# hlesmqh/WS3D

Measured on AMD Instinct MI355X. Metric: KITTI scenes/sec (16384 pts) Stage-1 RPN fwd, 1/2/4/8 GPU; FPS+group HBM GB/s, higher is better.
Workload: dtype f32

## Files before the change

### include/ws3d_ops.h

```cpp
#ifndef WS3D_OPS_H
#define WS3D_OPS_H

#include <stddef.h>
#include <stdint.h>

#ifdef __cplusplus
extern "C" {
#endif

#define WS3D_OK 0
#define WS3D_E_INVALID (-1)
#define WS3D_E_LAUNCH (-2)
#define WS3D_E_WORKSPACE (-3)
#define WS3D_E_UNSUPPORTED (-4)

#if defined(__GNUC__)
#define WS3D_API __attribute__((visibility("default")))
#else
#define WS3D_API
#endif

typedef void *ws3d_stream_t;

#define WS3D_ABI_VERSION 6
// ... 65 lines not shown
                  int32_t *idx, const void *sorted_known, ws3d_stream_t stream);

WS3D_API int ws3d_three_nn_weights(long rows, const float *dist2, float *weight, ws3d_stream_t stream);
WS3D_API int ws3d_three_nn_w(int b, int n, int m, const float *unknown, const float *known, float *dist2, int32_t *idx, float *weight,
                             const void *sorted_known, ws3d_stream_t stream);
WS3D_API int ws3d_three_nn_wq(int b, int n, int m, const float *unknown, const float *known, float *dist2, int32_t *idx, float *weight,
                              const void *sorted_known, const void *sorted_unknown, ws3d_stream_t stream);
WS3D_API int ws3d_three_nn_jobs(int b, int njobs, const int *n, const int *m, const float *const *unknown, const void *const *sorted_known,
                                float *const *dist2, int32_t *const *idx, float *const *weight, const void *const *sorted_unknown,
                                ws3d_stream_t stream);

WS3D_API int ws3d_pool_nsample(long rows, int nsample, const float *x, float *out, uint8_t *arg, ws3d_stream_t stream);
WS3D_API int ws3d_pool_nsample_grad(long rows, int nsample, const float *grad_out, const uint8_t *arg, float *grad_x,
                                    ws3d_stream_t stream);

WS3D_API int ws3d_gemm_pool(long rows, int nsample, int k_dim, int o_dim, const float *x_rows, const float *wt,
                            const float *bias, int relu, float *out, int out_stride, const int32_t *gate, long gate_limit, ws3d_stream_t stream);

WS3D_API int ws3d_gather_gemm(int b, int n, int m, int nsample, int c_feat, int o_dim, const float *feats, const float *xyz,
                     const float *new_xyz, const int32_t *nbr, const float *wt, const float *bias, int relu, float *out,
                     ws3d_stream_t stream);

WS3D_API int ws3d_gather_gemm2(int b, int n, int m, int nsample, int c_feat, int o1, int o2, const float *feats, const float *xyz,
                      const float *new_xyz, const int32_t *nbr, const float *w1t, const float *b1, int relu1, const float *w2t,
                      const float *b2, int relu2, float *out, ws3d_stream_t stream);

WS3D_API int ws3d_pgather_gemm2(int b, int n, int m, int nsample, int o1, int o2, const float *pmat, int p_stride, const float *xyz,
                       const float *new_xyz, const int32_t *nbr, const float *w1x, const float *b1, int relu1,
                       const float *w2t, const float *b2, int relu2, float *out, const int32_t *gate, long gate_limit, ws3d_stream_t stream);
WS3D_API int ws3d_pgather_rows(int b, int n, int m, int nsample, int o1, const float *pmat, int p_stride, const float *xyz, const float *new_xyz,
                      const int32_t *nbr, const float *w1x, const float *b1, int relu1, float *out, ws3d_stream_t stream);

WS3D_API int ws3d_qinterp_rows(int b, int n, int m, int o, const float *q, const int32_t *idx, const float *weight, const float *lin,
                      const float *skip, int c1, const float *wb, const float *bias, int relu, float *out, ws3d_stream_t stream);


WS3D_API int ws3d_compact_pairs(long centres, int nsample, const int32_t *nbr, int32_t *rowc, int32_t *rowsrc, int32_t *total, ws3d_stream_t stream);
WS3D_API int ws3d_compact_pairs_count(long centres, int nsample, const int32_t *nbr, int32_t *cnt, ws3d_stream_t stream);
WS3D_API int ws3d_compact_pairs_rows(long centres, int nsample, const int32_t *nbr, const int32_t *cnt, const int32_t *incl, int32_t *rowc,
                            int32_t *rowsrc, int32_t *total, ws3d_stream_t stream);
WS3D_API int ws3d_pgather_gemm2_compact(int b, int n, int m, long max_rows, int o1, int o2, const float *pmat, int p_stride, const float *xyz,
                               const float *new_xyz, const int32_t *rowc, const int32_t *rowsrc, const int32_t *total, const float *w1x,
                               const float *b1, int relu1, const float *w2t, const float *b2, int relu2, float *out, long limit, ws3d_stream_t stream);
WS3D_API int ws3d_pgather_gemm3_compact(int b, int n, int m, long max_rows, int o1, int o2, int o3, const float *pmat, int p_stride, const float *xyz,
                               const float *new_xyz, const int32_t *rowc, const int32_t *rowsrc, const int32_t *total, const float *w1x,
                               const float *b1, int relu1, const float *w2t, const float *b2, int relu2, const float *w3t, const float *b3,
                               float *out, int out_stride, long limit, ws3d_stream_t stream);
WS3D_API int ws3d_gemm_pool_compact(long max_rows, int k_dim, int o_dim, const float *x_rows, const int32_t *rowc, const int32_t *total,
                           const float *wt, const float *bias, float *out, int out_stride, long limit, ws3d_stream_t stream);
typedef struct ws3d_compact_mlp_args {
    int b, n, m;
    long max_rows;
    int o1, o2, o3;
    const float *pmat;
    int p_stride;
    const float *xyz, *new_xyz;
    const int32_t *rowc, *rowsrc, *total;
    const float *w1x, *b1;
    int relu1;
    const float *w2t, *b2;
    int relu2;
    const float *w3t, *b3;
    float *mid;
    float *out;
    int out_stride;
    long limit;
} ws3d_compact_mlp_args;
WS3D_API int ws3d_compact_mlp_pair(int kind, const ws3d_compact_mlp_args *scale0, const ws3d_compact_mlp_args *scale1, ws3d_stream_t stream);
WS3D_API int ws3d_chain_mlp3_ticket_ints(void);
WS3D_API size_t ws3d_chain_mlp3_blob_floats(int o2);
WS3D_API int ws3d_chain_mlp3_pack(const ws3d_compact_mlp_args *scale, float *blob, ws3d_stream_t stream);
WS3D_API int ws3d_chain_mlp3(const ws3d_compact_mlp_args *scale0, const ws3d_compact_mlp_args *scale1, const float *blob0, const float *blob1,
                             int32_t *ticket, int workgroups, ws3d_stream_t stream);

WS3D_API int ws3d_sa_mlp3_pool_compact(int b, int n, int m, long max_rows, int c1, int c2, int c3, const float *xyz, const float *new_xyz,
                              const float *feat, const int32_t *rowc, const int32_t *rowsrc, const int32_t *total, const float *w1t,
                              const float *b1, const float *w2t, const float *b2, const float *w3t, const float *b3, float *out,
                              int out_stride, long limit, ws3d_stream_t stream);

WS3D_API int ws3d_sa_mlp3_pool_lists(int b, int n, int m, int nsample, int c1, int c2, int c3, const float *xyz, const float *new_xyz,
                            const float *feat, const int32_t *nbr, const float *w1t, const float *b1, const float *w2t, const float *b2,
                            const float *w3t, const float *b3, int relu3, float *out, int out_stride, const int32_t *gate, long gate_limit,
                            ws3d_stream_t stream);

WS3D_API int ws3d_interp_gemm(int b, int n, int m, int c2, int c1, int o_dim, const float *known_feats, const float *unknown_feats,
                     const int32_t *idx, const float *weight, const float *wt, const float *bias, int relu, float *out,
                     ws3d_stream_t stream);

WS3D_API size_t ws3d_conv1x1_wgrad_workspace_bytes(int b, int o, int c, long l);
WS3D_API int ws3d_conv1x1_wgrad(int b, int o, int c, long l, const float *grad_out, const float *x, float *grad_w,
                                void *workspace, size_t workspace_bytes, ws3d_stream_t stream);

WS3D_API size_t ws3d_bn_workspace_bytes(int b, int c, long l);
WS3D_API int ws3d_bn_relu_train_fwd(int b, int c, long l, const float *x, const float *gamma, const float *beta, float eps,
                                    float momentum, int relu, float *running_mean, float *running_var,
                                    int64_t *num_batches_tracked, float *y, float *save_mean, float *save_invstd,
                                    void *workspace, size_t workspace_bytes, ws3d_stream_t stream);
WS3D_API int ws3d_bn_relu_train_bwd(int b, int c, long l, const float *x, const float *dy, const float *gamma,
                                    const float *beta, const float *save_mean, const float *save_invstd, int relu, float *dx,
                                    float *dgamma, float *dbeta, void *workspace, size_t workspace_bytes, ws3d_stream_t stream);

WS3D_API int ws3d_three_interpolate(int b, int c, int m, int n, const float *points, const int32_t *idx,
                           const float *weight, float *out, ws3d_stream_t stream);

WS3D_API int ws3d_three_interpolate_grad(int b, int c, int n, int m, const float *grad_out,
                                const int32_t *idx, const float *weight, float *grad_points,
                                ws3d_stream_t stream);

WS3D_API size_t ws3d_scatter_workspace_bytes(int b, int c, int n_targets, long slots_per_scene);
WS3D_API int ws3d_group_points_grad_det(int b, int c, int n, int npoints, int nsample, const float *grad_out,
                                        const int32_t *idx, float *grad_points, void *workspace,
                                        size_t workspace_bytes, ws3d_stream_t stream);
WS3D_API int ws3d_three_interpolate_grad_det(int b, int c, int n, int m, const float *grad_out, const int32_t *idx,
                                             const float *weight, float *grad_points, void *workspace,
                                             size_t workspace_bytes, ws3d_stream_t stream);

WS3D_API int ws3d_bias_act_inplace(int b, int o_ch, long l, int relu, float *y, const float *bias,
                                   ws3d_stream_t stream);

WS3D_API int ws3d_rowmax_bias_act(int b, int o_ch, long m, int s, int relu, const float *y, const float *bias,
                                  float *out, ws3d_stream_t stream);

WS3D_API int ws3d_query_and_group_nlc(int b, int n, int m, int c, float radius, int nsample, int use_xyz,
                                      const float *xyz, const float *new_xyz, const float *features_nlc,
                                      int32_t *idx_out, float *out_nlc, const void *sorted, ws3d_stream_t stream);
WS3D_API int ws3d_three_interpolate_nlc(int b, int c, int m, int n, const float *feats_nlc, const int32_t *idx,
                                        const float *weight, float *out_nlc, int out_stride, ws3d_stream_t stream);
WS3D_API int ws3d_rowmax_rows(long rows_out, int ns, int o_ch, const float *y, float *out, int out_stride,
                              ws3d_stream_t stream);

WS3D_API int ws3d_sa_mlp3_pool(long rows, int nsample, int c1, int c2, int c3, const float *x_rows4,
                               const float *w1t, const float *b1, const float *w2t, const float *b2,
                               const float *w3t, const float *b3, int relu3, float *out, int out_stride,
                               ws3d_stream_t stream);

WS3D_API int ws3d_mlp2_rows(long rows, int k_dim, int o1, int o2, const float *x_rows, const float *w1t, const float *b1, int relu1,
                   const float *w2t, const float *b2, int relu2, float *out, int *ticket, ws3d_stream_t stream);

WS3D_API size_t ws3d_rpn_heads_blob_bytes(int o2);
WS3D_API int ws3d_rpn_heads_pack(int o2, const float *w1t, const float *b1, int relu1, const float *w2t, const float *b2, int relu2, void *blob,
                        ws3d_stream_t stream);
WS3D_API int ws3d_rpn_heads(long rows, const float *x_rows, int heads, const void *blob_cls, float *out_cls, int *ticket_cls, int o2_reg,
                   const void *blob_reg, float *out_reg, int *ticket_reg, int workgroups, ws3d_stream_t stream);

WS3D_API size_t ws3d_gemm_rows_pack_bytes(int k_dim, int n_dim);
WS3D_API int ws3d_gemm_rows_pack(int k_dim, int n_dim, const float *wt, void *pack, ws3d_stream_t stream);
WS3D_API int ws3d_gemm_rows_split(long rows, int k_dim, int n_dim, const float *a, const void *pack, const float *bias, int relu, float *out,
                         ws3d_stream_t stream);

WS3D_API int ws3d_qinterp_gemm(int b, int n, int m, int c, int o_dim, const float *q, const int32_t *idx, const float *weight, const float *lin,
                      const float *skip, int c1, const float *wb, const float *b1, int relu1, const float *w2t, const float *b2, int relu2,
                      float *out, ws3d_stream_t stream);


WS3D_API int ws3d_boxes_overlap_bev(int num_a, const float *boxes_a, int num_b, const float *boxes_b,
                           float *ans, ws3d_stream_t stream);

WS3D_API int ws3d_boxes_iou_bev(int num_a, const float *boxes_a, int num_b, const float *boxes_b,
                       float *ans, ws3d_stream_t stream);

WS3D_API int ws3d_boxes_iou3d_paired(int n, const float *boxes_a, const float *boxes_b, float *overlap_bev, float *iou2d, float *iou3d,
                                     ws3d_stream_t stream);

WS3D_API int ws3d_nms_mask(int boxes_num, const float *boxes, float thresh, int normal, int full_grid,
                  uint64_t *mask, ws3d_stream_t stream);

WS3D_API size_t ws3d_nms_workspace_bytes(int boxes_num);
WS3D_API int ws3d_nms(int boxes_num, const float *boxes, float thresh, int normal, int max_keep,
                      void *workspace, size_t workspace_bytes, int64_t *keep, int32_t *num_keep,
                      ws3d_stream_t stream);

WS3D_API int ws3d_nms_batched(int batch, int boxes_num, const float *boxes, float thresh, int normal,
                              int max_keep, void *workspace, size_t workspace_bytes, int64_t *keep,
                              int32_t *num_keep, ws3d_stream_t stream);


WS3D_API int ws3d_radius_nms_batched(int batch, int n, const float *centers, float radius, int max_keep,
                                     void *workspace, size_t workspace_bytes, int64_t *keep,
                                     int32_t *num_keep, ws3d_stream_t stream);

WS3D_API int ws3d_topk_sorted(int b, int n, int k, const float *scores, float *out_scores, int64_t *out_idx,
                              ws3d_stream_t stream);
WS3D_API size_t ws3d_topk_workspace_bytes(int b, int n);
WS3D_API int ws3d_topk_sorted_ws(int b, int n, int k, const float *scores, float *out_scores, int64_t *out_idx, void *workspace,
                                 size_t workspace_bytes, ws3d_stream_t stream);
WS3D_API int ws3d_topk_sorted_sigmoid(int b, int n, int k, const float *logits, float *out_scores, int64_t *out_idx, ws3d_stream_t stream);
WS3D_API int ws3d_topk_sorted_sigmoid_ws(int b, int n, int k, const float *logits, float *out_scores, int64_t *out_idx, void *workspace,
                                         size_t workspace_bytes, ws3d_stream_t stream);

WS3D_API int ws3d_decode_center_boxes(int b, int n, int bins, float loc_scope, float loc_bin_size, float h, float w,
                                      float l, const float *xyz, const float *rpn_reg, float *boxes,
                                      ws3d_stream_t stream);

WS3D_API int ws3d_gather_boxes_bev(int b, int n, int top, const float *box, const int64_t *order, float *box_sorted, float *bev,
                          ws3d_stream_t stream);
WS3D_API int ws3d_decode_gather_boxes_bev(int b, int n, int top, int bins, float loc_scope, float loc_bin_size, float h, float w, float l,
                                          const float *xyz, const float *rpn_reg, const int64_t *order, float *box_sorted, float *bev,
                                          ws3d_stream_t stream);
WS3D_API int ws3d_select_proposals(int b, int top, int keep_stride, int k, const float *box_sorted, const float *scores_sorted,
                          const int64_t *keep, const int32_t *num, float extra_width, float *boxes_out, float *scores_out,
                          int64_t *count, float *pooled_boxes, ws3d_stream_t stream);
WS3D_API int ws3d_select_proposals_packed(int b, int top, int keep_stride, int k, const float *box_sorted, const float *scores_sorted,
                                          const int64_t *keep, const int32_t *num, float extra_width, float *boxes_out, float *scores_out,
                                          int64_t *count, float *pooled_boxes, float *packed, ws3d_stream_t stream);
WS3D_API int ws3d_select_proposals_send(int b, int top, int keep_stride, int k, const float *box_sorted, const float *scores_sorted,
                                        const int64_t *keep, const int32_t *num, float extra_width, float *boxes_out, float *scores_out,
                                        int64_t *count, float *pooled_boxes, float *send, long send_stride, ws3d_stream_t stream);
WS3D_API int ws3d_split_points_clear(long rows, int c, const float *pc, float *xyz, float *feats, void *clear, size_t clear_bytes,
                                     ws3d_stream_t stream);


WS3D_API int ws3d_roipool3d(int batch_size, int pts_num, int boxes_num, int feature_in_len,
                   int sampled_pts_num, const float *xyz, const float *boxes3d,
                   const float *pts_feature, float *pooled_features, int32_t *pooled_empty_flag,
                   int32_t *pts_idx, ws3d_stream_t stream);
WS3D_API int ws3d_roipool3d_fill(int batch_size, int pts_num, int boxes_num, int feature_in_len,
                   int sampled_pts_num, const float *xyz, const float *boxes3d,
                   const float *pts_feature, float *pooled_features, int32_t *pooled_empty_flag,
                   int32_t *pts_idx, ws3d_stream_t stream);

WS3D_API size_t ws3d_roipool3d_workspace_bytes(int batch_size, int pts_num);
WS3D_API int ws3d_roipool3d_ws(int batch_size, int pts_num, int boxes_num, int feature_in_len, int sampled_pts_num, const float *xyz,
                               const float *boxes3d, const float *pts_feature, float *pooled_features, int32_t *pooled_empty_flag,
                               int32_t *pts_idx, int fill, void *workspace, size_t workspace_bytes, ws3d_stream_t stream);


WS3D_API int ws3d_pts_in_boxes3d(int boxes_num, int pts_num, const float *pts, const float *boxes3d,
                        int64_t *flag, ws3d_stream_t stream);


WS3D_API int ws3d_instance_clouds(int batch, int pts_num, int centres_num, int feat_len, int sampled_pts_num, float radius, int mask_mode,
                                  float mask_thresh, const float *pts, const float *score, const float *feats, const float *centres,
                                  const int32_t *num, float *cloud, float *cloud_feats, int32_t *count, int32_t *pts_idx,
                                  ws3d_stream_t stream);
WS3D_API int ws3d_instance_clouds_count(int batch, int pts_num, int centres_num, float radius, const float *pts, const float *centres,
                                        const int32_t *num, int32_t *count, ws3d_stream_t stream);
WS3D_API int ws3d_instance_clouds_emit(int batch, int pts_num, int centres_num, int feat_len, float radius, int mask_mode, float mask_thresh,
                                       const float *pts, const float *score, const float *feats, const float *centres, const int32_t *num,
                                       const int64_t *offsets, float *rows, float *row_feats, int32_t *row_idx, ws3d_stream_t stream);


WS3D_API int ws3d_click_prepare(int batch, int pts_num, int clicks_num, int side, const float *offsets, float gauss_height, float gauss_status,
                                float gauss_cov, float centre_y, const float *pts, const float *clicks, const int32_t *num, float *score,
                                float *cand, int32_t *cand_num, ws3d_stream_t stream);



WS3D_API int ws3d_kitti_overlaps(int metric, int criterion, int frames, long max_pairs, const int32_t *gt_off, const int32_t *dt_off,
                                 const int64_t *out_off, const double *dt_boxes, const double *gt_boxes, double *out,
                                 ws3d_stream_t stream);

WS3D_API int ws3d_kitti_collect_scores(int frames, int max_dt, const int32_t *gt_off, const int32_t *dt_off, const int64_t *out_off,
                                       const double *overlaps, const int32_t *ignored_gt, const int32_t *ignored_dt,
                                       const double *dt_score, double min_overlap, double *tp_score, int32_t *tp_flag,
                                       ws3d_stream_t stream);

WS3D_API size_t ws3d_kitti_count_workspace_bytes(int frames, int num_thresh);
WS3D_API int ws3d_kitti_count(int metric, int frames, int max_dt, int num_thresh, const double *thresholds, const int32_t *gt_off,
                              const int32_t *dt_off, const int32_t *dc_off, const int64_t *out_off, const double *overlaps,
                              const int32_t *ignored_gt, const int32_t *ignored_dt, const double *dt_score, const double *dt_alpha,
                              const double *gt_alpha, const double *dt_bbox, const double *dc_bbox, double min_overlap, int compute_aos,
                              void *workspace, size_t workspace_bytes, double *pr, ws3d_stream_t stream);


WS3D_API int ws3d_stage2_embed(long rows, int pts_per_cloud, const float *pts, const float *box_ce, float extend, const float *wx0,
                               const float *bx0, const float *wx1, const float *bx1, const float *wf0, const float *bf0, const float *wf1,
                               const float *bf1, const float *wm, const float *bm, float *xyz_out, float *feat, ws3d_stream_t stream);
WS3D_API int ws3d_stage2_boxes(int rows, int loc_bins, int head_bins, float loc_scope, float h, float w, float l, const float *rcnn_reg,
                               float *pred_boxes3d, float *box_ce, ws3d_stream_t stream);
WS3D_API int ws3d_stage2_select(int batch, int slots, float cls_thresh, float iou_thresh, const float *size_window, float ground_y,
                                const float *box_ce, const float *rcnn_ref, const float *rcnn_cls, const float *rcnn_iou, const float *center,
                                const int32_t *num, float *boxes, int32_t *keep, float *key, ws3d_stream_t stream);

WS3D_API int ws3d_stage2_canonical_ragged(int rows, int clouds, const int32_t *offsets, const float *pts, const float *box_ce, float extend,
                                          float *pts_out, ws3d_stream_t stream);
WS3D_API int ws3d_furthest_point_sampling_ragged_gather(int clouds, const int32_t *offsets, const int32_t *sizes_host, int m, const float *xyz,
                                                        int32_t *idx, float *new_xyz, ws3d_stream_t stream);
WS3D_API int ws3d_ball_query_ragged(int clouds, const int32_t *offsets, int m, float radius, int nsample, const float *xyz, const float *new_xyz,
                                    int global_rows, int32_t *idx, ws3d_stream_t stream);

WS3D_API int ws3d_stage2_rcnn_loss(int rows, int loc_bins, int head_bins, float loc_scope, float h, float w, float l, const float *rcnn_cls,
                                   const float *rcnn_reg, const float *pred_boxes3d, const float *gt_boxes, const float *cls, float *vals,
                                   int32_t *counts, float *grad_cls, float *grad_reg, ws3d_stream_t stream);
WS3D_API int ws3d_stage2_ioun_loss(int rows, const float *rcnn_iou, const float *rcnn_ref, const float *pred_boxes3d, const float *refined_box,
                                   const float *gt_boxes, const float *cls, float *vals, int32_t *counts, float *grad_iou, float *grad_ref,
                                   ws3d_stream_t stream);

WS3D_API int ws3d_rpn_center_labels(int batch, int n, int kmax, int pts_stride, float gauss_height, float gauss_status, double gauss_cov,
                                    const float *pts, const float *centres, const int32_t *count, float *cls_label, float *reg_label,
                                    ws3d_stream_t stream);
WS3D_API size_t ws3d_rpn_loss_workspace_bytes(int rows);
WS3D_API int ws3d_rpn_loss(int rows, int bins, double loc_scope, double loc_bin_size, double alpha, double gamma, double weight_cls,
                           double weight_reg, const float *rpn_cls, const float *rpn_reg, const float *cls_label, const float *reg_label,
                           float *vals, int32_t *counts, float *grad_cls, float *grad_reg, void *workspace, size_t workspace_bytes,
                           ws3d_stream_t stream);

WS3D_API int ws3d_scan_prepare_limit(void);
WS3D_API size_t ws3d_scan_prepare_workspace_bytes(int scenes, long total_points);
WS3D_API int ws3d_scan_prepare(int scenes, const int32_t *offsets, long total_points, int max_scan_points, const float *raw, const float *calib,
                               const int32_t *img_hw, const float *scope, int npoints, uint64_t seed, const int64_t *scene_key, int key_bits,
                               float *pts_input, int32_t *src_index, int32_t *valid_count, int32_t *status, void *workspace,
                               size_t workspace_bytes, ws3d_stream_t stream);

WS3D_API int ws3d_stage2_batch_param_bytes(void);
WS3D_API int ws3d_stage2_batch(int samples, const void *params, const float *rows, const int32_t *offsets, int records, long total_rows,
                               int key_bits, float *cur_box_point, float *cur_box_reflect, float *train_mask, int32_t *status,
// ... 14 lines not shown
```

### ws3d_amd/_lib.py

```python
from __future__ import annotations

import ctypes as C
import os

_HERE = os.path.dirname(os.path.abspath(__file__))
DIST_MODE = int(os.environ.get("WS3D_DIST_MODE", "0") or 0)
LIB_PATH = os.environ.get("WS3D_HIP_LIB") or os.path.join(
    _HERE, "libws3d_hip.so" if DIST_MODE == 0 else "libws3d_hip_dm%d.so" % DIST_MODE)

E_INVALID, E_LAUNCH, E_WORKSPACE, E_UNSUPPORTED = -1, -2, -3, -4
ABI_VERSION = 6

_vp = C.c_void_p
_i = C.c_int
_f = C.c_float
_sz = C.c_size_t

class CompactMlpArgs(C.Structure):
    _fields_ = [("b", _i), ("n", _i), ("m", _i), ("max_rows", C.c_long), ("o1", _i), ("o2", _i), ("o3", _i), ("pmat", _vp), ("p_stride", _i),
                ("xyz", _vp), ("new_xyz", _vp), ("rowc", _vp), ("rowsrc", _vp), ("total", _vp), ("w1x", _vp), ("b1", _vp), ("relu1", _i),
                ("w2t", _vp), ("b2", _vp), ("relu2", _i), ("w3t", _vp), ("b3", _vp), ("mid", _vp), ("out", _vp), ("out_stride", _i), ("limit", C.c_long)]


SIGNATURES = {
    "ws3d_abi_version": (_i, []),
    "ws3d_tune": (_i, [_i, _i]),
    "ws3d_dist_mode": (_i, []),
    "ws3d_last_error": (C.c_char_p, []),
    "ws3d_device_info": (_i, [C.c_char_p, _i, C.POINTER(_i), C.POINTER(_i)]),
    "ws3d_furthest_point_sampling": (_i, [_i, _i, _i, _vp, _vp, _vp, _vp]),
    "ws3d_furthest_point_sampling_gather": (_i, [_i, _i, _i, _vp, _vp, _vp, _vp, _vp]),
    "ws3d_furthest_point_sampling_nested": (_i, [_i, _i, _i, _vp, _vp, _vp, _vp]),
    "ws3d_furthest_point_sampling_nested_chain": (_i, [_i, _i, _i, _vp, _vp, _vp, _vp, _vp]),
    "ws3d_fps_ragged_limit": (_i, []),
    "ws3d_furthest_point_sampling_ragged": (_i, [_i, _vp, _vp, _i, _vp, _vp, _vp]),
    "ws3d_fps_workspace_bytes": (_sz, [_i, _i]),
    "ws3d_furthest_point_sampling_ws": (_i, [_i, _i, _i, _vp, _vp, _vp, _vp, _vp, _sz, _vp]),
    "ws3d_gather_points": (_i, [_i, _i, _i, _i, _vp, _vp, _vp, _vp]),
    "ws3d_gather_points_grad": (_i, [_i, _i, _i, _i, _vp, _vp, _vp, _vp]),
    "ws3d_ball_query": (_i, [_i, _i, _i, _f, _i, _vp, _vp, _vp, _vp, _vp]),
    "ws3d_ball_query_fill": (_i, [_i, _i, _i, _f, _i, _vp, _vp, _vp, _vp, _vp]),
    "ws3d_ball_query_pairs": (_i, [_i, _i, _i, _f, _i, _vp, _vp, _vp, _vp, _vp, _vp, _vp, _vp]),
    "ws3d_ball_query_pairs2": (_i, [_i, _i, _i, _vp, _vp, _vp, C.c_float, _i, _vp, _vp, _vp, _vp, C.c_float, _i, _vp, _vp, _vp, _vp, _vp]),
    "ws3d_sorted_points_bytes": (_sz, [_i, _i]),
    "ws3d_sort_points_x": (_i, [_i, _i, _vp, _vp, _vp]),
    "ws3d_sort_points_xz": (_i, [_i, _i, _vp, _vp, _vp]),
    "ws3d_sort_points_grid": (_i, [_i, _i, _vp, _vp, _vp]),
    "ws3d_sort_points_jobs": (_i, [_i, _i, _vp, _vp, _vp, _vp, _vp]),
    "ws3d_group_points": (_i, [_i, _i, _i, _i, _i, _vp, _vp, _vp, _vp]),
    "ws3d_group_points_grad": (_i, [_i, _i, _i, _i, _i, _vp, _vp, _vp, _vp]),
    "ws3d_query_and_group": (_i, [_i, _i, _i, _i, _f, _i, _i, _vp, _vp, _vp, _vp, _vp, _vp, _vp]),
    "ws3d_three_nn": (_i, [_i, _i, _i, _vp, _vp, _vp, _vp, _vp, _vp]),
    "ws3d_three_interpolate": (_i, [_i, _i, _i, _i, _vp, _vp, _vp, _vp, _vp]),
    "ws3d_three_interpolate_grad": (_i, [_i, _i, _i, _i, _vp, _vp, _vp, _vp, _vp]),
    "ws3d_bn_workspace_bytes": (C.c_size_t, [_i, _i, C.c_long]),
    "ws3d_bn_relu_train_fwd": (_i, [_i, _i, C.c_long, _vp, _vp, _vp, C.c_float, C.c_float, _i, _vp, _vp, _vp, _vp, _vp, _vp,
                                    _vp, C.c_size_t, _vp]),
    "ws3d_bn_relu_train_bwd": (_i, [_i, _i, C.c_long, _vp, _vp, _vp, _vp, _vp, _vp, _i, _vp, _vp, _vp, _vp, C.c_size_t, _vp]),
    "ws3d_conv1x1_wgrad_workspace_bytes": (C.c_size_t, [_i, _i, _i, C.c_long]),
    "ws3d_conv1x1_wgrad": (_i, [_i, _i, _i, C.c_long, _vp, _vp, _vp, _vp, C.c_size_t, _vp]),
    "ws3d_gemm_pool": (_i, [C.c_long, _i, _i, _i, _vp, _vp, _vp, _i, _vp, _i, _vp, C.c_long, _vp]),
    "ws3d_pool_nsample": (_i, [C.c_long, _i, _vp, _vp, _vp, _vp]),
    "ws3d_pool_nsample_grad": (_i, [C.c_long, _i, _vp, _vp, _vp, _vp]),
    "ws3d_scatter_workspace_bytes": (C.c_size_t, [_i, _i, _i, C.c_long]),
    "ws3d_group_points_grad_det": (_i, [_i, _i, _i, _i, _i, _vp, _vp, _vp, _vp, C.c_size_t, _vp]),
    "ws3d_three_interpolate_grad_det": (_i, [_i, _i, _i, _i, _vp, _vp, _vp, _vp, _vp, C.c_size_t, _vp]),
    "ws3d_query_and_group_nlc": (_i, [_i, _i, _i, _i, _f, _i, _i, _vp, _vp, _vp, _vp, _vp, _vp, _vp]),
    "ws3d_three_interpolate_nlc": (_i, [_i, _i, _i, _i, _vp, _vp, _vp, _vp, _i, _vp]),
    "ws3d_rowmax_rows": (_i, [C.c_long, _i, _i, _vp, _vp, _i, _vp]),
    "ws3d_sa_mlp3_pool": (_i, [C.c_long, _i, _i, _i, _i, _vp, _vp, _vp, _vp, _vp, _vp, _vp, _i, _vp, _i, _vp]),
    "ws3d_qinterp_gemm": (_i, [_i, _i, _i, _i, _i, _vp, _vp, _vp, _vp, _vp, _i, _vp, _vp, _i, _vp, _vp, _i, _vp, _vp]),
    "ws3d_mlp2_rows": (_i, [C.c_long, _i, _i, _i, _vp, _vp, _vp, _i, _vp, _vp, _i, _vp, _vp, _vp]),
    "ws3d_rpn_heads_blob_bytes": (_sz, [_i]),
    "ws3d_rpn_heads_pack": (_i, [_i, _vp, _vp, _i, _vp, _vp, _i, _vp, _vp]),
    "ws3d_rpn_heads": (_i, [C.c_long, _vp, _i, _vp, _vp, _vp, _i, _vp, _vp, _vp, _i, _vp]),
    "ws3d_gemm_rows_pack_bytes": (_sz, [_i, _i]),
    "ws3d_gemm_rows_pack": (_i, [_i, _i, _vp, _vp, _vp]),
    "ws3d_gemm_rows_split": (_i, [C.c_long, _i, _i, _vp, _vp, _vp, _i, _vp, _vp]),
    "ws3d_decode_center_boxes": (_i, [_i, _i, _i, _f, _f, _f, _f, _f, _vp, _vp, _vp, _vp]),
    "ws3d_topk_sorted": (_i, [_i, _i, _i, _vp, _vp, _vp, _vp]),
    "ws3d_topk_workspace_bytes": (C.c_size_t, [_i, _i]),
    "ws3d_topk_sorted_ws": (_i, [_i, _i, _i, _vp, _vp, _vp, _vp, C.c_size_t, _vp]),
    "ws3d_topk_sorted_sigmoid": (_i, [_i, _i, _i, _vp, _vp, _vp, _vp]),
    "ws3d_topk_sorted_sigmoid_ws": (_i, [_i, _i, _i, _vp, _vp, _vp, _vp, C.c_size_t, _vp]),
    "ws3d_three_nn_weights": (_i, [C.c_long, _vp, _vp, _vp]),
    "ws3d_three_nn_w": (_i, [_i, _i, _i, _vp, _vp, _vp, _vp, _vp, _vp, _vp]),
    "ws3d_three_nn_wq": (_i, [_i, _i, _i, _vp, _vp, _vp, _vp, _vp, _vp, _vp, _vp]),
    "ws3d_three_nn_jobs": (_i, [_i, _i, _vp, _vp, _vp, _vp, _vp, _vp, _vp, _vp, _vp]),
    "ws3d_bias_act_inplace": (_i, [_i, _i, C.c_long, _i, _vp, _vp, _vp]),
    "ws3d_rowmax_bias_act": (_i, [_i, _i, C.c_long, _i, _i, _vp, _vp, _vp, _vp]),
    "ws3d_boxes_overlap_bev": (_i, [_i, _vp, _i, _vp, _vp, _vp]),
    "ws3d_boxes_iou_bev": (_i, [_i, _vp, _i, _vp, _vp, _vp]),
    "ws3d_boxes_iou3d_paired": (_i, [_i, _vp, _vp, _vp, _vp, _vp, _vp]),
    "ws3d_nms_mask": (_i, [_i, _vp, _f, _i, _i, _vp, _vp]),
    "ws3d_nms_workspace_bytes": (_sz, [_i]),
    "ws3d_nms": (_i, [_i, _vp, _f, _i, _i, _vp, _sz, _vp, _vp, _vp]),
    "ws3d_nms_batched": (_i, [_i, _i, _vp, _f, _i, _i, _vp, _sz, _vp, _vp, _vp]),
    "ws3d_radius_nms_batched": (_i, [_i, _i, _vp, _f, _i, _vp, _sz, _vp, _vp, _vp]),
    "ws3d_gather_gemm": (_i, [_i, _i, _i, _i, _i, _i, _vp, _vp, _vp, _vp, _vp, _vp, _i, _vp, _vp]),
    "ws3d_gather_gemm2": (_i, [_i, _i, _i, _i, _i, _i, _i, _vp, _vp, _vp, _vp, _vp, _vp, _i, _vp, _vp, _i, _vp, _vp]),
    "ws3d_pgather_gemm2": (_i, [_i, _i, _i, _i, _i, _i, _vp, _i, _vp, _vp, _vp, _vp, _vp, _i, _vp, _vp, _i, _vp, _vp, C.c_long, _vp]),
    "ws3d_pgather_rows": (_i, [_i, _i, _i, _i, _i, _vp, _i, _vp, _vp, _vp, _vp, _vp, _i, _vp, _vp]),
    "ws3d_qinterp_rows": (_i, [_i, _i, _i, _i, _vp, _vp, _vp, _vp, _vp, _i, _vp, _vp, _i, _vp, _vp]),
    "ws3d_compact_pairs": (_i, [C.c_long, _i, _vp, _vp, _vp, _vp, _vp]),
    "ws3d_compact_pairs_count": (_i, [C.c_long, _i, _vp, _vp, _vp]),
    "ws3d_compact_pairs_rows": (_i, [C.c_long, _i, _vp, _vp, _vp, _vp, _vp, _vp, _vp]),
    "ws3d_pgather_gemm2_compact": (_i, [_i, _i, _i, C.c_long, _i, _i, _vp, _i, _vp, _vp, _vp, _vp, _vp, _vp, _vp, _i, _vp, _vp, _i, _vp, C.c_long, _vp]),
    "ws3d_pgather_gemm3_compact": (_i, [_i, _i, _i, C.c_long, _i, _i, _i, _vp, _i, _vp, _vp, _vp, _vp, _vp, _vp, _vp, _i, _vp, _vp, _i, _vp, _vp, _vp, _i, C.c_long, _vp]),
    "ws3d_gemm_pool_compact": (_i, [C.c_long, _i, _i, _vp, _vp, _vp, _vp, _vp, _vp, _i, C.c_long, _vp]),
    "ws3d_compact_mlp_pair": (_i, [_i, C.POINTER(CompactMlpArgs), C.POINTER(CompactMlpArgs), _vp]),
    "ws3d_chain_mlp3_ticket_ints": (_i, []),
    "ws3d_chain_mlp3_blob_floats": (_sz, [_i]),
    "ws3d_chain_mlp3_pack": (_i, [C.POINTER(CompactMlpArgs), _vp, _vp]),
    "ws3d_chain_mlp3": (_i, [C.POINTER(CompactMlpArgs), C.POINTER(CompactMlpArgs), _vp, _vp, _vp, _i, _vp]),
    "ws3d_sa_mlp3_pool_compact": (_i, [_i, _i, _i, C.c_long, _i, _i, _i, _vp, _vp, _vp, _vp, _vp, _vp, _vp, _vp, _vp, _vp, _vp, _vp, _vp, _i, C.c_long, _vp]),
    "ws3d_sa_mlp3_pool_lists": (_i, [_i, _i, _i, _i, _i, _i, _i, _vp, _vp, _vp, _vp, _vp, _vp, _vp, _vp, _vp, _vp, _i, _vp, _i, _vp, C.c_long, _vp]),
    "ws3d_interp_gemm": (_i, [_i, _i, _i, _i, _i, _i, _vp, _vp, _vp, _vp, _vp, _vp, _i, _vp, _vp]),
    "ws3d_gather_boxes_bev": (_i, [_i, _i, _i, _vp, _vp, _vp, _vp, _vp]),
    "ws3d_select_proposals": (_i, [_i, _i, _i, _i, _vp, _vp, _vp, _vp, _f, _vp, _vp, _vp, _vp, _vp]),
    "ws3d_decode_gather_boxes_bev": (_i, [_i, _i, _i, _i, _f, _f, _f, _f, _f, _vp, _vp, _vp, _vp, _vp, _vp]),
    "ws3d_select_proposals_packed": (_i, [_i, _i, _i, _i, _vp, _vp, _vp, _vp, _f, _vp, _vp, _vp, _vp, _vp, _vp]),
    "ws3d_select_proposals_send": (_i, [_i, _i, _i, _i, _vp, _vp, _vp, _vp, _f, _vp, _vp, _vp, _vp, _vp, C.c_long, _vp]),
    "ws3d_split_points_clear": (_i, [C.c_long, _i, _vp, _vp, _vp, _vp, C.c_size_t, _vp]),
    "ws3d_roipool3d": (_i, [_i, _i, _i, _i, _i, _vp, _vp, _vp, _vp, _vp, _vp, _vp]),
    "ws3d_roipool3d_fill": (_i, [_i, _i, _i, _i, _i, _vp, _vp, _vp, _vp, _vp, _vp, _vp]),
    "ws3d_roipool3d_workspace_bytes": (C.c_size_t, [_i, _i]),
    "ws3d_roipool3d_ws": (_i, [_i, _i, _i, _i, _i, _vp, _vp, _vp, _vp, _vp, _vp, _i, _vp, C.c_size_t, _vp]),
    "ws3d_pts_in_boxes3d": (_i, [_i, _i, _vp, _vp, _vp, _vp]),
    "ws3d_instance_clouds": (_i, [_i, _i, _i, _i, _i, _f, _i, _f, _vp, _vp, _vp, _vp, _vp, _vp, _vp, _vp, _vp, _vp]),
    "ws3d_instance_clouds_count": (_i, [_i, _i, _i, _f, _vp, _vp, _vp, _vp, _vp]),
    "ws3d_instance_clouds_emit": (_i, [_i, _i, _i, _i, _f, _i, _f, _vp, _vp, _vp, _vp, _vp, _vp, _vp, _vp, _vp, _vp]),
    "ws3d_click_prepare": (_i, [_i, _i, _i, _i, _vp, _f, _f, _f, _f, _vp, _vp, _vp, _vp, _vp, _vp, _vp]),
    "ws3d_kitti_overlaps": (_i, [_i, _i, _i, C.c_long, _vp, _vp, _vp, _vp, _vp, _vp, _vp]),
    "ws3d_kitti_collect_scores": (_i, [_i, _i, _vp, _vp, _vp, _vp, _vp, _vp, _vp, C.c_double, _vp, _vp, _vp]),
    "ws3d_kitti_count_workspace_bytes": (_sz, [_i, _i]),
    "ws3d_kitti_count": (_i, [_i, _i, _i, _i, _vp, _vp, _vp, _vp, _vp, _vp, _vp, _vp, _vp, _vp, _vp, _vp, _vp, C.c_double, _i, _vp,
                              _sz, _vp, _vp]),
    "ws3d_stage2_embed": (_i, [C.c_long, _i, _vp, _vp, _f] + [_vp] * 10 + [_vp, _vp, _vp]),
    "ws3d_stage2_boxes": (_i, [_i, _i, _i, _f, _f, _f, _f, _vp, _vp, _vp, _vp]),
    "ws3d_stage2_select": (_i, [_i, _i, _f, _f, C.POINTER(_f), _f, _vp, _vp, _vp, _vp, _vp, _vp, _vp, _vp, _vp, _vp]),
    "ws3d_stage2_canonical_ragged": (_i, [_i, _i, _vp, _vp, _vp, _f, _vp, _vp]),
    "ws3d_furthest_point_sampling_ragged_gather": (_i, [_i, _vp, _vp, _i, _vp, _vp, _vp, _vp]),
    "ws3d_ball_query_ragged": (_i, [_i, _vp, _i, _f, _i, _vp, _vp, _i, _vp, _vp]),
    "ws3d_stage2_rcnn_loss": (_i, [_i, _i, _i, _f, _f, _f, _f] + [_vp] * 9 + [_vp]),
    "ws3d_stage2_ioun_loss": (_i, [_i] + [_vp] * 10 + [_vp]),
    "ws3d_rpn_center_labels": (_i, [_i, _i, _i, _i, _f, _f, C.c_double] + [_vp] * 5 + [_vp]),
    "ws3d_rpn_loss_workspace_bytes": (_sz, [_i]),
    "ws3d_rpn_loss": (_i, [_i, _i] + [C.c_double] * 6 + [_vp] * 8 + [_vp, _sz, _vp]),
    "ws3d_scan_prepare_limit": (_i, []),
    "ws3d_scan_prepare_workspace_bytes": (_sz, [_i, C.c_long]),
    "ws3d_scan_prepare": (_i, [_i, _vp, C.c_long, _i, _vp, _vp, _vp, _vp, _i, C.c_uint64, _vp, _i, _vp, _vp, _vp, _vp, _vp, _sz, _vp]),
    "ws3d_stage2_batch_param_bytes": (_i, []),
    "ws3d_stage2_batch": (_i, [_i, _vp, _vp, _vp, _i, C.c_long, _i, _vp, _vp, _vp, _vp, _vp]),
    "ws3d_roipool3d_plan": (_i, [_i, _i, _i, _i, _i, _i, _sz]),
    "ws3d_ball_query_plan": (_i, [_i, _i, _i, _i, _i, _i, _i, _i, _i, _i, _i, _vp]),
}


class Ws3dError(RuntimeError):
    pass


_lib = None


def load() -> C.CDLL:
    global _lib
    if _lib is not None:
        return _lib
    if not os.path.exists(LIB_PATH):
        raise Ws3dError(
            f"{LIB_PATH} is missing: the MI355X HIP library has not been built "
            "(run `python -m ws3d_amd.build`).  ws3d_amd has no CPU fallback.")
    import torch
    try:
        lib = C.CDLL(LIB_PATH)
    except OSError as e:
        raise Ws3dError(f"cannot load {LIB_PATH}: {e}") from e
    for name, (res, args) in SIGNATURES.items():
        fn = getattr(lib, name)
        fn.restype = res
        fn.argtypes = args
    if lib.ws3d_abi_version() != ABI_VERSION:
        raise Ws3dError(f"{LIB_PATH} exports ABI version {lib.ws3d_abi_version()}, this package binds version {ABI_VERSION}: "
                        "rebuild it (`python -m ws3d_amd.build`)")
    if not os.environ.get("WS3D_HIP_LIB") and lib.ws3d_dist_mode() != DIST_MODE:
        raise Ws3dError(f"{LIB_PATH} was built with WS3D_DIST_MODE={lib.ws3d_dist_mode()}, expected {DIST_MODE}: rebuild it")
    _lib = lib
    return lib


def check(rc: int, what: str = "") -> None:
    if rc != 0:
        msg = load().ws3d_last_error()
        raise Ws3dError(f"{what or 'ws3d'} failed (rc={rc}): {msg.decode() if msg else ''}")
```

### ws3d_amd/build.py

```python
from __future__ import annotations

import argparse
import concurrent.futures as cf
import glob
import os
import shutil
import subprocess
import sys

HERE = os.path.dirname(os.path.abspath(__file__))
CSRC = os.path.join(HERE, "csrc")
OBJ = os.path.join(CSRC, "build")
LIB = os.path.join(HERE, "libws3d_hip.so")
DIST_MODES = (0, 1, 2)


def lib_path(dist_mode: int = 0) -> str:
    return LIB if dist_mode == 0 else os.path.join(HERE, "libws3d_hip_dm%d.so" % dist_mode)
ARCH = "gfx950"
SOURCES = ["core.hip", "fps.hip", "fps_v3.hip", "fps_bucket.hip", "fps_nested.hip", "fps_ragged.hip", "fps_pruned.hip", "ballquery_group.hip", "interpolate.hip", "roipool3d.hip", "iou3d.hip", "proposals.hip", "scatter_det.hip", "sa_mlp.hip", "bn_relu.hip", "gemm_pool.hip", "conv_wgrad.hip", "chain_mlp.hip", "rpn_heads.hip", "gemm_rows.hip", "kitti_eval.hip", "instance_clouds.hip", "click.hip", "stage2.hip", "stage2_ragged.hip", "stage2_loss.hip", "rpn_targets.hip", "scan_prepare.hip", "stage2_batch.hip"]
CXXFLAGS = ["-O3", "-std=c++17", "-fPIC", "-ffp-contract=off", "-fno-fast-math",
            "-fvisibility=hidden", "-Wall", "-Wno-unused-function"]


def hipcc() -> str:
    for cand in (os.environ.get("HIPCC"), shutil.which("hipcc"), "/opt/rocm/bin/hipcc"):
        if cand and os.path.exists(cand):
            return cand
    raise RuntimeError("hipcc not found (looked at $HIPCC, PATH, /opt/rocm/bin)")


def _deps(src: str):
    return [src, *glob.glob(os.path.join(CSRC, "*.h")), os.path.join(HERE, "..", "include", "ws3d_ops.h"),
            os.path.join(CSRC, "exports.map"), os.path.abspath(__file__)]


def _compile(src: str, force: bool, verbose: bool, dist_mode: int = 0) -> str:
    path = os.path.join(CSRC, src)
    obj = os.path.join(OBJ if dist_mode == 0 else OBJ + "_dm%d" % dist_mode, os.path.splitext(src)[0] + ".o")
    if not force and os.path.exists(obj) and all(
            os.path.getmtime(obj) >= os.path.getmtime(d) for d in _deps(path)):
        return obj
    cmd = [hipcc(), f"--offload-arch={ARCH}", *CXXFLAGS, f"-DWS3D_DIST_MODE={dist_mode}", *os.environ.get("WS3D_EXTRA_DEFS", "").split(), "-c", path, "-o", obj]
    if verbose:
        print(" ".join(cmd), flush=True)
    r = subprocess.run(cmd, capture_output=True, text=True)
    if r.returncode != 0:
        raise RuntimeError(f"hipcc failed for {src}:\n{r.stdout}\n{r.stderr}")
    if verbose and r.stderr.strip():
        print(r.stderr)
    return obj


def build(force: bool = False, verbose: bool = False, dist_mode: int = 0) -> str:
    LIB = lib_path(dist_mode)
    os.makedirs(OBJ if dist_mode == 0 else OBJ + "_dm%d" % dist_mode, exist_ok=True)
    with cf.ThreadPoolExecutor(max_workers=min(len(SOURCES), os.cpu_count() or 4, 16)) as ex:
        objs = list(ex.map(lambda s: _compile(s, force, verbose, dist_mode), SOURCES))
    if force or not os.path.exists(LIB) or any(os.path.getmtime(o) > os.path.getmtime(LIB) for o in objs):
        cmd = [hipcc(), f"--offload-arch={ARCH}", "-shared", "-fPIC", "-Wl,--version-script=" + os.path.join(CSRC, "exports.map"), "-o", LIB, *objs]
        if verbose:
            print(" ".join(cmd), flush=True)
        r = subprocess.run(cmd, capture_output=True, text=True)
        if r.returncode != 0:
            raise RuntimeError(f"link failed:\n{r.stdout}\n{r.stderr}")
    return LIB


def rebuild_one(src: str, verbose: bool = False) -> str:
    _compile(src, True, verbose)
    objs = [os.path.join(OBJ, os.path.splitext(s_)[0] + ".o") for s_ in SOURCES]
    missing = [o for o in objs if not os.path.exists(o)]
    if missing:
        return build(False, verbose)
    cmd = [hipcc(), f"--offload-arch={ARCH}", "-shared", "-fPIC", "-Wl,--version-script=" + os.path.join(CSRC, "exports.map"), "-o", LIB, *objs]
    r = subprocess.run(cmd, capture_output=True, text=True)
    if r.returncode != 0:
        raise RuntimeError(f"link failed:\n{r.stdout}\n{r.stderr}")
    return LIB


if __name__ == "__main__":
    ap = argparse.ArgumentParser()
    ap.add_argument("--force", action="store_true")
    ap.add_argument("--verbose", action="store_true")
    ap.add_argument("--dist-mode", type=int, default=0, choices=DIST_MODES)
    ap.add_argument("--all-dist-modes", action="store_true")
    ap.add_argument("--only", default=None, help="recompile this one source (forced) and relink")
    a = ap.parse_args()
    if a.only:
        print(rebuild_one(a.only, a.verbose))
        sys.exit(0)
    for dm in (DIST_MODES if a.all_dist_modes else (a.dist_mode,)):
        print(build(a.force, a.verbose, dm))
    sys.exit(0)
```

### ws3d_amd/compat.py

```python
from __future__ import annotations

import sys
import types

import os

import torch

from . import _lib
from ._lib import Ws3dError, check


def _dev(*tensors):
    dev = None
    for t in tensors:
        if t is None:
            continue
        if not t.is_cuda:
            raise Ws3dError("ws3d_amd ops need HIP ('cuda') tensors; there is no CPU fallback")
        if not t.is_contiguous():
            raise Ws3dError("ws3d_amd ops need contiguous tensors (the reference asserts the same)")
        if dev is None:
            dev = t.device
        elif t.device != dev:
# ... 388 lines not shown
    b, c = x.size(0), x.size(1)
    l = x.numel() // max(b * c, 1)
    y = torch.empty_like(x)
    mean = torch.empty((c,), dtype=torch.float32, device=dev)
    invstd = torch.empty((c,), dtype=torch.float32, device=dev)
    lib = _lib.load()
    nbytes = lib.ws3d_bn_workspace_bytes(b, c, l)
    ws = torch.empty((nbytes + 7) // 8, dtype=torch.float64, device=dev)
    with _on(dev):
        check(lib.ws3d_bn_relu_train_fwd(b, c, l, _p(x), _p(gamma), _p(beta), float(eps), float(momentum), int(bool(relu)),
                                         _p(running_mean), _p(running_var), _p(num_batches_tracked), _p(y), _p(mean), _p(invstd), _p(ws), nbytes,
                                         _stream()), "bn_relu_train_fwd")
    return y, mean, invstd


def bn_relu_train_bwd(x, dy, gamma, beta, save_mean, save_invstd, relu=True):
    dev = _dev(x, dy, gamma, beta, save_mean, save_invstd)
    _f32(x, "x"); _f32(dy, "dy")
    b, c = x.size(0), x.size(1)
    l = x.numel() // max(b * c, 1)
    dx = torch.empty_like(x)
    dgamma = torch.empty((c,), dtype=torch.float32, device=dev)
    dbeta = torch.empty((c,), dtype=torch.float32, device=dev)
    lib = _lib.load()
    nbytes = lib.ws3d_bn_workspace_bytes(b, c, l)
    ws = torch.empty((nbytes + 7) // 8, dtype=torch.float64, device=dev)
    with _on(dev):
        check(lib.ws3d_bn_relu_train_bwd(b, c, l, _p(x), _p(dy), _p(gamma), _p(beta), _p(save_mean), _p(save_invstd),
                                         int(bool(relu)), _p(dx), _p(dgamma), _p(dbeta), _p(ws), nbytes, _stream()),
              "bn_relu_train_bwd")
    return dx, dgamma, dbeta


def conv1x1_wgrad(grad_out, x, shape=None):
    dev = _dev(grad_out, x)
    _f32(grad_out, "grad_out"); _f32(x, "x")
    b, o, c = x.size(0), grad_out.size(1), x.size(1)
    l = x.numel() // max(b * c, 1)
    if grad_out.numel() != b * o * l:
        raise Ws3dError("conv1x1_wgrad: grad_out and x disagree in shape")
    gw = torch.empty((o, c) if shape is None else tuple(shape), dtype=torch.float32, device=dev)
    lib = _lib.load()
    nbytes = lib.ws3d_conv1x1_wgrad_workspace_bytes(b, o, c, l)
    ws = torch.empty((nbytes + 3) // 4, dtype=torch.float32, device=dev)
    with _on(dev):
        check(lib.ws3d_conv1x1_wgrad(b, o, c, l, _p(grad_out), _p(x), _p(gw), _p(ws), nbytes, _stream()), "conv1x1_wgrad")
    return gw


def _gate(gate):
    if gate is None:
        return None, 0
    total, limit = gate
    return total.data_ptr(), int(limit)


def gemm_pool(x_rows, wt, bias, relu, nsample, out, col0=0, gate=None):
    dev = _dev(x_rows, wt, bias)
    _f32(x_rows, "x_rows"); _f32(wt, "wt")
    rows, k = x_rows.shape
    o = wt.size(1)
    if rows % 64 or rows // 64 > 65535 or o % 64 or k % 4 or nsample not in (16, 32) or wt.size(0) != k:
        return False
    view = out[:, col0:col0 + o]
    with _on(dev):
        check(_lib.load().ws3d_gemm_pool(rows, nsample, k, o, _p(x_rows), _p(wt), _p(bias), int(bool(relu)), view.data_ptr(),
                                         out.size(1), *_gate(gate), _stream()), "gemm_pool")
    return True


def gather_gemm(feats, xyz, new_xyz, nbr, wt_feat_then_xyz, bias, relu):
    dev = _dev(feats, xyz, new_xyz, nbr, wt_feat_then_xyz)
    _f32(feats, "feats"); _f32(xyz, "xyz"); _f32(new_xyz, "new_xyz"); _i32(nbr, "nbr"); _f32(wt_feat_then_xyz, "wt")
    B, N, C = feats.shape
    M, ns = nbr.size(1), nbr.size(2)
    O = wt_feat_then_xyz.size(1)
    rows = B * M * ns
    if C % 4 or O % 64 or rows % 64 or rows // 64 > 65535 or wt_feat_then_xyz.size(0) != C + 3 or not feats.is_contiguous():
        return None
    out = torch.empty((rows, O), dtype=torch.float32, device=dev)
    with _on(dev):
        check(_lib.load().ws3d_gather_gemm(B, N, M, ns, C, O, _p(feats), _p(xyz), _p(new_xyz), _p(nbr), _p(wt_feat_then_xyz), _p(bias),
                                           int(bool(relu)), _p(out), _stream()), "gather_gemm")
    return out


def gather_gemm2(feats, xyz, new_xyz, nbr, w1t_feat_then_xyz, b1, relu1, w2t, b2, relu2):
    dev = _dev(feats, xyz, new_xyz, nbr, w1t_feat_then_xyz, w2t)
    _f32(feats, "feats"); _f32(xyz, "xyz"); _f32(new_xyz, "new_xyz"); _i32(nbr, "nbr"); _f32(w1t_feat_then_xyz, "w1t"); _f32(w2t, "w2t")
    B, N, C = feats.shape
    M, ns = nbr.size(1), nbr.size(2)
    O1, O2 = w1t_feat_then_xyz.size(1), w2t.size(1)
    rows = B * M * ns
    if (C % 4 or O1 not in (64, 128, 256) or O2 % 4 or rows % 64 or w1t_feat_then_xyz.size(0) != C + 3 or w2t.size(0) != O1 or
            not feats.is_contiguous() or not w2t.is_contiguous() or not w1t_feat_then_xyz.is_contiguous()):
        return None
    out = torch.empty((rows, O2), dtype=torch.float32, device=dev)
    with _on(dev):
        check(_lib.load().ws3d_gather_gemm2(B, N, M, ns, C, O1, O2, _p(feats), _p(xyz), _p(new_xyz), _p(nbr), _p(w1t_feat_then_xyz), _p(b1),
                                            int(bool(relu1)), _p(w2t), _p(b2), int(bool(relu2)), _p(out), _stream()), "gather_gemm2")
    return out


def pgather_gemm2(pmat, col0, o1, xyz, new_xyz, nbr, w1x, b1, relu1, w2t, b2, relu2, out=None, gate=None):
    dev = _dev(pmat, xyz, new_xyz, nbr, w1x, w2t)
    _f32(pmat, "pmat"); _f32(xyz, "xyz"); _f32(new_xyz, "new_xyz"); _i32(nbr, "nbr"); _f32(w1x, "w1x"); _f32(w2t, "w2t")
    B, N = xyz.size(0), xyz.size(1)
    M, ns = nbr.size(1), nbr.size(2)
    O2 = w2t.size(1)
    if (o1 not in (64, 128) or O2 % 4 or (M * ns) % 64 or pmat.dim() != 2 or pmat.size(0) != B * N or pmat.stride(1) != 1 or
            col0 < 0 or col0 + o1 > pmat.size(1) or tuple(w1x.shape) != (3, o1) or w2t.size(0) != o1 or not w1x.is_contiguous() or not w2t.is_contiguous()):
        return None
    if out is None:
        out = torch.empty((B * M * ns, O2), dtype=torch.float32, device=dev)
    elif tuple(out.shape) != (B * M * ns, O2) or not out.is_contiguous():
        raise ValueError("pgather_gemm2: out must be a contiguous (B*M*ns, O2) tensor")
    with _on(dev):
        check(_lib.load().ws3d_pgather_gemm2(B, N, M, ns, o1, O2, pmat.data_ptr() + 4 * col0, pmat.stride(0), _p(xyz), _p(new_xyz), _p(nbr), _p(w1x), _p(b1),
                                             int(bool(relu1)), _p(w2t), _p(b2), int(bool(relu2)), _p(out), *_gate(gate), _stream()), "pgather_gemm2")
    return out


def pgather_rows(pmat, col0, o1, xyz, new_xyz, nbr, w1x, b1, relu1):
    dev = _dev(pmat, xyz, new_xyz, nbr, w1x)
    _f32(pmat, "pmat"); _f32(xyz, "xyz"); _f32(new_xyz, "new_xyz"); _i32(nbr, "nbr"); _f32(w1x, "w1x")
    B, N = xyz.size(0), xyz.size(1)
    M, ns = nbr.size(1), nbr.size(2)
    if (o1 % 4 or col0 % 4 or pmat.dim() != 2 or pmat.size(0) != B * N or pmat.stride(1) != 1 or pmat.stride(0) % 4 or col0 < 0 or
            col0 + o1 > pmat.size(1) or tuple(w1x.shape) != (3, o1) or not w1x.is_contiguous() or pmat.data_ptr() % 16):
        return None
    out = torch.empty((B * M * ns, o1), dtype=torch.float32, device=dev)
    with _on(dev):
        check(_lib.load().ws3d_pgather_rows(B, N, M, ns, o1, pmat.data_ptr() + 4 * col0, pmat.stride(0), _p(xyz), _p(new_xyz), _p(nbr), _p(w1x), _p(b1),
                                            int(bool(relu1)), _p(out), _stream()), "pgather_rows")
    return out


def qinterp_rows(q, idx, weight, lin=None, skip=None, wb=None, bias=None, relu=True):
    dev = _dev(q, idx, weight)
    _f32(q, "q"); _i32(idx, "idx"); _f32(weight, "weight")
    B, M, O = q.shape
    N = idx.size(1)
    c1 = 0 if skip is None else skip.size(2)
    if (O % 4 or not q.is_contiguous() or (lin is None and c1 > 4) or (lin is not None and (tuple(lin.shape) != (B * N, O) or not lin.is_contiguous())) or
            (lin is None and c1 > 0 and (wb is None or tuple(wb.shape) != (c1, O) or not wb.is_contiguous() or not skip.is_contiguous()))):
        return None
    out = torch.empty((B * N, O), dtype=torch.float32, device=dev)
    with _on(dev):
        check(_lib.load().ws3d_qinterp_rows(B, N, M, O, _p(q), _p(idx), _p(weight), _p(lin), _p(skip), c1, _p(wb), _p(bias), int(bool(relu)), _p(out),
                                            _stream()), "qinterp_rows")
    return out


def qinterp_gemm(q, idx, weight, w2t, b2, relu2, lin=None, skip=None, wb=None, bias=None, relu=True):
    dev = _dev(q, idx, weight, w2t)
    _f32(q, "q"); _i32(idx, "idx"); _f32(weight, "weight"); _f32(w2t, "w2t")
    B, M, C = q.shape
    N = idx.size(1)
    O = w2t.size(1)
    c1 = 0 if skip is None else skip.size(2)
    if ((B * N) % 64 or C % 16 or O % 128 or w2t.size(0) != C or not q.is_contiguous() or not w2t.is_contiguous() or not idx.is_contiguous() or
            not weight.is_contiguous() or (lin is None and c1 > 4) or (lin is not None and (tuple(lin.shape) != (B * N, C) or not lin.is_contiguous())) or
            (lin is None and c1 > 0 and (wb is None or tuple(wb.shape) != (c1, C) or not wb.is_contiguous() or not skip.is_contiguous()))):
        return None
    out = torch.empty((B * N, O), dtype=torch.float32, device=dev)
    with _on(dev):
        check(_lib.load().ws3d_qinterp_gemm(B, N, M, C, O, _p(q), _p(idx), _p(weight), _p(lin), _p(skip), c1, _p(wb), _p(bias), int(bool(relu)), _p(w2t),
                                            _p(b2), int(bool(relu2)), _p(out), _stream()), "qinterp_gemm")
    return out


def compact_pairs(nbr, ordered=False):
    if not ordered:
        dev = _dev(nbr)
        _i32(nbr, "nbr")
        B, M, ns = nbr.shape
        rowc = torch.empty(B * M * ns, dtype=torch.int32, device=dev)
        rowsrc = torch.empty(B * M * ns, dtype=torch.int32, device=dev)
        total = torch.zeros(1, dtype=torch.int32, device=dev)
        with _on(dev):
            check(_lib.load().ws3d_compact_pairs(B * M, ns, _p(nbr), _p(rowc), _p(rowsrc), _p(total), _stream()), "compact_pairs")
        return rowc, rowsrc, total
    dev = _dev(nbr)
    _i32(nbr, "nbr")
    B, M, ns = nbr.shape
    centres = B * M
    cnt = torch.empty(centres, dtype=torch.int32, device=dev)
    rowc = torch.empty(centres * ns, dtype=torch.int32, device=dev)
    rowsrc = torch.empty(centres * ns, dtype=torch.int32, device=dev)
    total = torch.empty(1, dtype=torch.int32, device=dev)
    with _on(dev):
        lib = _lib.load()
        check(lib.ws3d_compact_pairs_count(centres, ns, _p(nbr), _p(cnt), _stream()), "compact_pairs_count")
        incl = torch.cumsum(cnt, dim=0, dtype=torch.int32)
        check(lib.ws3d_compact_pairs_rows(centres, ns, _p(nbr), _p(cnt), _p(incl), _p(rowc), _p(rowsrc), _p(total), _stream()), "compact_pairs_rows")
    return rowc, rowsrc, total


def pgather_gemm2_compact(pmat, col0, o1, xyz, new_xyz, pairs, w1x, b1, relu1, w2t, b2, relu2, limit=-1):
    rowc, rowsrc, total = pairs
    dev = _dev(pmat, xyz, new_xyz, rowc, w1x, w2t)
    _f32(pmat, "pmat"); _f32(xyz, "xyz"); _f32(new_xyz, "new_xyz"); _f32(w1x, "w1x"); _f32(w2t, "w2t")
    B, N = xyz.size(0), xyz.size(1)
    M = new_xyz.size(1)
    O2 = w2t.size(1)
    rows = rowc.numel()
    if (o1 not in (64, 128, 256) or O2 % 4 or pmat.dim() != 2 or pmat.size(0) != B * N or pmat.stride(1) != 1 or col0 < 0 or col0 + o1 > pmat.size(1) or
            tuple(w1x.shape) != (3, o1) or w2t.size(0) != o1 or not w1x.is_contiguous() or not w2t.is_contiguous()):
        return None
    out = torch.empty((rows, O2), dtype=torch.float32, device=dev)
    with _on(dev):
        check(_lib.load().ws3d_pgather_gemm2_compact(B, N, M, rows, o1, O2, pmat.data_ptr() + 4 * col0, pmat.stride(0), _p(xyz), _p(new_xyz), _p(rowc),
                                                     _p(rowsrc), _p(total), _p(w1x), _p(b1), int(bool(relu1)), _p(w2t), _p(b2), int(bool(relu2)), _p(out),
                                                     int(limit), _stream()), "pgather_gemm2_compact")
    return out


def pgather_gemm3_compact(pmat, col0, o1, xyz, new_xyz, pairs, w1x, b1, relu1, w2t, b2, relu2, w3t, b3, out2d, col_offset, limit=-1, max_lds=160 * 1024):
    rowc, rowsrc, total = pairs
    dev = _dev(pmat, xyz, new_xyz, rowc, w1x, w2t, w3t, out2d)
    _f32(pmat, "pmat"); _f32(xyz, "xyz"); _f32(new_xyz, "new_xyz"); _f32(w1x, "w1x"); _f32(w2t, "w2t"); _f32(w3t, "w3t"); _f32(out2d, "out2d")
    B, N = xyz.size(0), xyz.size(1)
    M = new_xyz.size(1)
    O2, O3 = w2t.size(1), w3t.size(1)
    rows = rowc.numel()
    lds = 4 * ((o1 + (O2 + 15) // 16 * 16) * 65 + 2 * 16 * 64)
    if (o1 not in (64, 128) or O2 % 4 or O3 % 128 or lds > min(max_lds, 160 * 1024 - 1024) or pmat.dim() != 2 or pmat.size(0) != B * N or pmat.stride(1) != 1 or
            col0 < 0 or col0 + o1 > pmat.size(1) or tuple(w1x.shape) != (3, o1) or w2t.size(0) != o1 or w3t.size(0) != O2 or not w1x.is_contiguous() or
            not w2t.is_contiguous() or not w3t.is_contiguous() or out2d.dim() != 2 or out2d.stride(1) != 1 or col_offset < 0 or col_offset + O3 > out2d.size(1)):
        return False
    with _on(dev):
        check(_lib.load().ws3d_pgather_gemm3_compact(B, N, M, rows, o1, O2, O3, pmat.data_ptr() + 4 * col0, pmat.stride(0), _p(xyz), _p(new_xyz), _p(rowc),
                                                     _p(rowsrc), _p(total), _p(w1x), _p(b1), int(bool(relu1)), _p(w2t), _p(b2), int(bool(relu2)), _p(w3t), _p(b3),
                                                     out2d.data_ptr() + 4 * col_offset, out2d.stride(0), int(limit), _stream()), "pgather_gemm3_compact")
    return True


def gemm_pool_compact(x_rows, pairs, wt, bias, out2d, col_offset, limit=-1):
    rowc, rowsrc, total = pairs
    dev = _dev(x_rows, rowc, wt, out2d)
    _f32(x_rows, "x_rows"); _f32(wt, "wt"); _f32(out2d, "out2d")
    rows, k = x_rows.shape
    o = wt.size(1)
    if (k % 4 or o % 64 or wt.size(0) != k or rows != rowc.numel() or not x_rows.is_contiguous() or not wt.is_contiguous() or out2d.dim() != 2 or
            out2d.stride(1) != 1 or col_offset < 0 or col_offset + o > out2d.size(1)):
        return False
    with _on(dev):
        check(_lib.load().ws3d_gemm_pool_compact(rows, k, o, _p(x_rows), _p(rowc), _p(total), _p(wt), _p(bias), out2d.data_ptr() + 4 * col_offset,
                                                 out2d.stride(0), int(limit), _stream()), "gemm_pool_compact")
    return True


def compact_mlp_pair(kind, scales, max_lds=160 * 1024, mids=None):
    import ctypes as C
    if len(scales) != 2 or scales[0]["o1"] != scales[1]["o1"]:
        return None if kind == 2 else False
    blocks, keep, outs = [], [], []
    for si, a in enumerate(scales):
        rowc, rowsrc, total = a["pairs"]
        pmat, xyz, new_xyz, w1x, w2t, w3t, out2d, o1, col0, col = a["pmat"], a["xyz"], a["new_xyz"], a["w1x"], a["w2t"], a["w3t"], a["out2d"], a["o1"], a["col0"], a["col_offset"]
        dev = _dev(pmat, xyz, new_xyz, rowc, w1x, w2t, w3t, out2d)
        for t_, nm in ((pmat, "pmat"), (xyz, "xyz"), (new_xyz, "new_xyz"), (w1x, "w1x"), (w2t, "w2t"), (w3t, "w3t"), (out2d, "out2d")):
            _f32(t_, nm)
        B, N, M = xyz.size(0), xyz.size(1), new_xyz.size(1)
        O2, O3 = w2t.size(1), w3t.size(1)
        rows = rowc.numel()
        lds3 = 4 * ((o1 + (O2 + 15) // 16 * 16) * 65 + 2 * 16 * 64)
        ok = (O2 % 4 == 0 and pmat.dim() == 2 and pmat.size(0) == B * N and pmat.stride(1) == 1 and col0 >= 0 and col0 + o1 <= pmat.size(1) and
              tuple(w1x.shape) == (3, o1) and w2t.size(0) == o1 and w3t.size(0) == O2 and w1x.is_contiguous() and w2t.is_contiguous() and w3t.is_contiguous() and
              out2d.dim() == 2 and out2d.stride(1) == 1 and col >= 0 and col + O3 <= out2d.size(1))
        if kind == 3:
            ok = ok and o1 in (64, 128) and O3 % 128 == 0 and lds3 <= min(max_lds, 160 * 1024 - 1024)
        elif kind == 2:
            ok = ok and o1 in (64, 128, 256)
        else:
            ok = ok and O3 % 64 == 0 and mids is not None and tuple(mids[si].shape) == (rows, O2) and mids[si].is_contiguous()
        if not ok:
            return None if kind == 2 else False
        mid = mids[si] if kind == 1 else (torch.empty((rows, O2), dtype=torch.float32, device=dev) if kind == 2 else None)
        outs.append(mid)
        keep.append((pmat, xyz, new_xyz, rowc, rowsrc, total, w1x, w2t, w3t, out2d, mid, a["b1"], a["b2"], a["b3"]))
        blocks.append(_lib.CompactMlpArgs(B, N, M, rows, o1, O2, O3, pmat.data_ptr() + 4 * col0, pmat.stride(0), _p(xyz), _p(new_xyz), _p(rowc), _p(rowsrc),
                                          _p(total), _p(w1x), _p(a["b1"]), int(bool(a["relu1"])), _p(w2t), _p(a["b2"]), int(bool(a["relu2"])), _p(w3t), _p(a["b3"]),
                                          _p(mid), out2d.data_ptr() + 4 * col, out2d.stride(0), -1))
    with _on(dev):
        rc = _lib.load().ws3d_compact_mlp_pair(int(kind), C.byref(blocks[0]), C.byref(blocks[1]), _stream())
    if rc == _lib.E_UNSUPPORTED:
        return None if kind == 2 else False
    check(rc, "compact_mlp_pair")
    return outs if kind == 2 else True


CHAIN_WORKGROUPS = 0
TUNE_KEYS = {"chain_wgs": 0, "mlp2_wgs": 1, "sa1_wgs": 2, "fp_wgs": 3, "pair_wgs": 4, "bq_wide_nw": 5}


def tune(name: str, value: int = -1) -> int:
    rc = _lib.load().ws3d_tune(TUNE_KEYS[name], int(value))
    if rc < 0:
        check(rc, "tune")
    return rc


_CHAIN_BLOBS = {}


def chain_ticket_ints() -> int:
    return int(_lib.load().ws3d_chain_mlp3_ticket_ints())


def _chain_blob(block, tensors, dev):
    import ctypes as C
    key = tuple((t.data_ptr(), t._version) if t is not None else None for t in tensors)
    hit = _CHAIN_BLOBS.get(key)
    if hit is None:
        n = int(_lib.load().ws3d_chain_mlp3_blob_floats(block.o2))
        blob = torch.empty(n, dtype=torch.float32, device=dev)
        with _on(dev):
            check(_lib.load().ws3d_chain_mlp3_pack(C.byref(block), _p(blob), _stream()), "chain_mlp3_pack")
        if torch.cuda.is_current_stream_capturing():
            return blob
# ... 955 lines not shown
```

### ws3d_amd/csrc/gemm_pool.hip

```cpp
#include <cstdlib>

#include "common.h"
#include "compact_pool.h"
#include "mfma_tile.h"

namespace ws3d {

template <int NS, int MB, int NB>
__global__ __launch_bounds__(256) void gemm_pool_big_kernel(int k_dim, int o_dim, const float *__restrict__ x,
                                                            const float *__restrict__ wt, const float *__restrict__ bias,
                                                            int relu, float *__restrict__ out, int out_stride, int xcd,
                                                            const int32_t *__restrict__ gate, long gate_limit) {
    if (gate && (long)*gate <= gate_limit) return;
    constexpr int TM = 64 * MB, TN = 64 * NB;
    __shared__ float xs[2][GP_KT][TM + 1];
    __shared__ __attribute__((aligned(16))) float ws[2][GP_KT][TN];
    const Wave w;
    long row_tile;
    int col_tile;
    gg_tile<false>(o_dim / TN, xcd, blockIdx.x, row_tile, col_tile);
    const long row0 = row_tile * TM;
    const int col0 = col_tile * TN;
    RowsA<MB> load_a;
    load_a.k_dim = k_dim;
#pragma unroll
    for (int i = 0; i < MB; ++i) load_a.p[i] = x + (row0 + (w.tid >> 2) + 64 * i) * (long)k_dim;
    floatx16 acc[MB][NB];
    mfma_k_loop<MB, NB, false>(w, acc, xs, ws, k_dim, load_a, wt, o_dim, col0);
#pragma unroll
    for (int i = 0; i < MB; ++i)
#pragma unroll
        for (int j = 0; j < NB; ++j)
            pool_rows<NS>(w, acc[i][j], bias, relu, out, out_stride, row0 + sub_row<MB>(w, i), col0 + sub_col<NB, false>(w, j) + w.l32);
}

struct GatherA {
    const float *frow, *prow, *crow;
    int c_feat;
    __device__ __forceinline__ GatherA(long r, int c_feat_, int n, int m, int ns, const float *__restrict__ feats, const float *__restrict__ xyz,
                                       const float *__restrict__ new_xyz, const int32_t *__restrict__ nbr) {
        const long cm = r / ns;
        const long b = cm / m;
        const int src = nbr[r];
        frow = feats + ((size_t)b * n + (size_t)src) * c_feat_;
        prow = xyz + ((size_t)b * n + (size_t)src) * 3;
        crow = new_xyz + (size_t)cm * 3;
        c_feat = c_feat_;
    }
    __device__ __forceinline__ float4 operator()(int, int k) const {
        if (k < c_feat) return *reinterpret_cast<const float4 *>(frow + k);
        if (k == c_feat) return make_float4(prow[0] - crow[0], prow[1] - crow[1], prow[2] - crow[2], 0.f);
        return f4_zero();
    }
};

__global__ __launch_bounds__(256) void gather_gemm_kernel(int c_feat, int o_dim, int n, int m, int ns, const float *__restrict__ feats,
                                                          const float *__restrict__ xyz, const float *__restrict__ new_xyz,
                                                          const int32_t *__restrict__ nbr, const float *__restrict__ wt,
                                                          const float *__restrict__ bias, int relu, float *__restrict__ out, int tps) {
    __shared__ float xs[2][GP_KT][GP_XS];
    __shared__ __attribute__((aligned(16))) float ws[2][GP_KT][64];
    const Wave w;
    long row_tile;
    int col_tile;
    gg_tile<true>(o_dim / 64, tps, blockIdx.x, row_tile, col_tile);
    const long row0 = row_tile * 64;
    const int col0 = col_tile * 64;
    const GatherA load_a(row0 + (w.tid >> 2), c_feat, n, m, ns, feats, xyz, new_xyz, nbr);
    floatx16 acc[1][1];
    mfma_k_loop<1, 1, false>(w, acc, xs, ws, c_feat + 3, load_a, wt, o_dim, col0);
    store_rows(w, acc[0][0], bias, relu, out, o_dim, row0 + w.wm * 32, col0 + w.bc);
}

template <int NB1>
__global__ __launch_bounds__(256) void gather_gemm2_kernel(int c_feat, int o2, int n, int m, int ns, const float *__restrict__ feats,
                                                           const float *__restrict__ xyz, const float *__restrict__ new_xyz,
                                                           const int32_t *__restrict__ nbr, const float *__restrict__ w1t,
                                                           const float *__restrict__ b1, int relu1, const float *__restrict__ w2t,
                                                           const float *__restrict__ b2, int relu2, float *__restrict__ out) {
    constexpr int O1 = NB1 * 64;
    extern __shared__ __attribute__((aligned(16))) float smem2[];
    auto &xs = *reinterpret_cast<float (*)[2][GP_KT][GP_XS]>(smem2);
    auto &w1s = *reinterpret_cast<float (*)[2][GP_KT][O1]>(smem2 + 2 * GP_KT * GP_XS);
    float *act = smem2, *w2s = smem2 + O1 * GP_XS;
    const Wave w;
    const long row0 = (long)blockIdx.x * 64;
    const GatherA load_a(row0 + (w.tid >> 2), c_feat, n, m, ns, feats, xyz, new_xyz, nbr);
    floatx16 acc1[1][NB1];
    mfma_k_loop<1, NB1, true>(w, acc1, xs, w1s, c_feat + 3, load_a, w1t, O1, 0);
#pragma unroll
    for (int j = 0; j < NB1; ++j) store_act(w, acc1[0][j], b1, relu1, act, j * 64 + w.bc);
    lds_layer<1>(w, act, O1 / GP_KT, w2t, O1, o2, w2s, 0, 1, [&](const floatx16 &acc, int col) __attribute__((always_inline)) {
        if (col < o2) store_rows(w, acc, b2, relu2, out, o2, row0 + w.wm * 32, col);
    });
}

template <int NB1>
__global__ __launch_bounds__(256) void pgather_gemm2_kernel(int o2, int n, int m, int ns, const float *__restrict__ pmat, int p_stride,
                                                            const float *__restrict__ xyz, const float *__restrict__ new_xyz,
                                                            const int32_t *__restrict__ nbr, const float *__restrict__ w1x,
                                                            const float *__restrict__ b1, int relu1, const float *__restrict__ w2t,
                                                            const float *__restrict__ b2, int relu2, float *__restrict__ out,
                                                            const int32_t *__restrict__ gate, long gate_limit) {
    if (gate && (long)*gate <= gate_limit) return;
    constexpr int O1 = NB1 * 64;
    extern __shared__ __attribute__((aligned(16))) float smem2[];
    float *act = smem2, *w2s = smem2 + O1 * GP_XS;
    const Wave w;
    const long row0 = (long)blockIdx.x * 64;
    const long scene = row0 / ((long)m * ns);
    ppoint_layer1<NB1>(w, [&](int tr) __attribute__((always_inline)) { return PairRow{scene, (row0 + tr) / ns, nbr[row0 + tr]}; }, n, pmat, p_stride, xyz, new_xyz, w1x, b1, relu1, act);
    lds_layer<1>(w, act, O1 / GP_KT, w2t, O1, o2, w2s, 0, 1, [&](const floatx16 &acc, int col) __attribute__((always_inline)) {
        if (col < o2) store_rows(w, acc, b2, relu2, out, o2, row0 + w.wm * 32, col);
    });
}

__global__ __launch_bounds__(256) void pgather_rows_kernel(long rows, int o1, int n, int m, int ns, const float *__restrict__ pmat, int p_stride,
                                                           const float *__restrict__ xyz, const float *__restrict__ new_xyz,
                                                           const int32_t *__restrict__ nbr, const float *__restrict__ w1x,
                                                           const float *__restrict__ b1, int relu1, float *__restrict__ out) {
    const int q4 = o1 >> 2;
    const long total = rows * q4;
    for (long e = (long)blockIdx.x * 256 + threadIdx.x; e < total; e += (long)gridDim.x * 256) {
        const long r = e / q4;
        const int c4 = (int)(e - r * q4) * 4;
        const long cm = r / ns, scene = cm / m;
        const int src = nbr[r];
        const float *pr = xyz + ((size_t)scene * n + (size_t)src) * 3, *cr = new_xyz + (size_t)cm * 3;
        const float dx = pr[0] - cr[0], dy = pr[1] - cr[1], dz = pr[2] - cr[2];
        const float4 pv = *reinterpret_cast<const float4 *>(pmat + ((size_t)scene * n + (size_t)src) * p_stride + c4);
        const float4 wx = *reinterpret_cast<const float4 *>(w1x + c4), wy = *reinterpret_cast<const float4 *>(w1x + o1 + c4),
                     wz = *reinterpret_cast<const float4 *>(w1x + 2 * o1 + c4);
        const float4 bv = b1 ? *reinterpret_cast<const float4 *>(b1 + c4) : make_float4(0.f, 0.f, 0.f, 0.f);
        float4 y;
        y.x = __builtin_fmaf(dz, wz.x, __builtin_fmaf(dy, wy.x, __builtin_fmaf(dx, wx.x, pv.x))) + bv.x;
        y.y = __builtin_fmaf(dz, wz.y, __builtin_fmaf(dy, wy.y, __builtin_fmaf(dx, wx.y, pv.y))) + bv.y;
        y.z = __builtin_fmaf(dz, wz.z, __builtin_fmaf(dy, wy.z, __builtin_fmaf(dx, wx.z, pv.z))) + bv.z;
        y.w = __builtin_fmaf(dz, wz.w, __builtin_fmaf(dy, wy.w, __builtin_fmaf(dx, wx.w, pv.w))) + bv.w;
        if (relu1) { y.x = y.x < 0.f ? 0.f : y.x; y.y = y.y < 0.f ? 0.f : y.y; y.z = y.z < 0.f ? 0.f : y.z; y.w = y.w < 0.f ? 0.f : y.w; }
        *reinterpret_cast<float4 *>(out + r * (long)o1 + c4) = y;
    }
}

__global__ __launch_bounds__(256) void pair_count_kernel(long centres, int ns, const int32_t *__restrict__ nbr, int32_t *__restrict__ cnt) {
    const long c = (long)blockIdx.x * 256 + threadIdx.x;
    if (c >= centres) return;
    const int32_t *row = nbr + c * ns;
    int k = 1, prev = row[0];
    for (int s2 = 1; s2 < ns; ++s2) { const int v = row[s2]; k += v > prev; prev = v; }
    cnt[c] = k;
}

__global__ __launch_bounds__(256) void pair_rows_kernel(long centres, int ns, const int32_t *__restrict__ nbr, const int32_t *__restrict__ cnt,
                                                        const int32_t *__restrict__ incl, int32_t *__restrict__ rowc, int32_t *__restrict__ rowsrc,
                                                        int32_t *__restrict__ total) {
    const long e = (long)blockIdx.x * 256 + threadIdx.x;
    if (e >= centres * ns) return;
// ... 30 lines not shown
        for (int s2 = 0; s2 < k; ++s2) { rowc[first + s2] = (int32_t)c; rowsrc[first + s2] = row[s2]; }
    }
}

struct CompactSrc {
    const int32_t *__restrict__ rowc, *__restrict__ rowsrc;
    long row0, T;
    int m;
    __device__ __forceinline__ PairRow operator()(int tr) const {
        const long t = min(row0 + tr, T - 1);
        const int cm = rowc[t];
        return PairRow{cm / m, cm, rowsrc[t]};
    }
};

template <int NB1>
__device__ __forceinline__ void pgather_gemm2_compact_body(const unsigned bx, const unsigned by, const unsigned gy, int o2, int n, int m,
                                                           const float *__restrict__ pmat, int p_stride,
                                                           const float *__restrict__ xyz, const float *__restrict__ new_xyz,
                                                           const int32_t *__restrict__ rowc, const int32_t *__restrict__ rowsrc,
                                                           const int32_t *__restrict__ total, const float *__restrict__ w1x,
                                                           const float *__restrict__ b1, int relu1, const float *__restrict__ w2t,
                                                           const float *__restrict__ b2, int relu2, float *__restrict__ out, long limit) {
    constexpr int O1 = NB1 * 64;
    const long T = *total;
    const long row0 = (long)bx * 64;
    if (row0 >= T || (limit >= 0 && T > limit)) return;
    extern __shared__ __attribute__((aligned(16))) float smem2[];
    float *act = smem2, *w2s = smem2 + O1 * GP_XS;
    const Wave w;
    ppoint_layer1<NB1>(w, CompactSrc{rowc, rowsrc, row0, T, m}, n, pmat, p_stride, xyz, new_xyz, w1x, b1, relu1, act);
    lds_layer<1>(w, act, O1 / GP_KT, w2t, O1, o2, w2s, (int)by, (int)gy, [&](const floatx16 &acc, int col) __attribute__((always_inline)) {
        if (col < o2) store_rows(w, acc, b2, relu2, out, o2, row0 + w.wm * 32, col, T);
    });
}

template <int NB1>
__global__ __launch_bounds__(256) void pgather_gemm2_compact_kernel(int o2, int n, int m, const float *__restrict__ pmat, int p_stride,
                                                                    const float *__restrict__ xyz, const float *__restrict__ new_xyz,
                                                                    const int32_t *__restrict__ rowc, const int32_t *__restrict__ rowsrc,
                                                                    const int32_t *__restrict__ total, const float *__restrict__ w1x,
                                                                    const float *__restrict__ b1, int relu1, const float *__restrict__ w2t,
                                                                    const float *__restrict__ b2, int relu2, float *__restrict__ out, long limit) {
    pgather_gemm2_compact_body<NB1>(blockIdx.x, blockIdx.y, gridDim.y, o2, n, m, pmat, p_stride, xyz, new_xyz, rowc, rowsrc, total, w1x, b1, relu1, w2t, b2,
                                    relu2, out, limit);
}

struct CompactMlpArgs {
    const float *pmat, *xyz, *new_xyz;
    const int32_t *rowc, *rowsrc, *total;
    const float *w1x, *b1, *w2t, *b2, *w3t, *b3;
    float *mid, *out;
    long limit;
    int o2, o3, n, m, p_stride, relu1, relu2, out_stride, gy, pad;
};

template <int NB1>
__global__ __launch_bounds__(256) void pgather_gemm2_compact_pair_kernel(const CompactMlpArgs a0, const CompactMlpArgs a1, const unsigned split,
                                                                         const unsigned total_x) {
    for (unsigned bx = blockIdx.x; bx < total_x; bx += gridDim.x) {
        const bool second = bx >= split;
        const CompactMlpArgs &a = second ? a1 : a0;
        if (blockIdx.y < (unsigned)a.gy)
            pgather_gemm2_compact_body<NB1>(second ? bx - split : bx, blockIdx.y, (unsigned)a.gy, a.o2, a.n, a.m, a.pmat, a.p_stride, a.xyz, a.new_xyz,
                                            a.rowc, a.rowsrc, a.total, a.w1x, a.b1, a.relu1, a.w2t, a.b2, a.relu2, a.mid, a.limit);
        __syncthreads();
    }
}

__device__ __forceinline__ void gemm_pool_compact_body(const unsigned bx, int k_dim, int o_dim, const float *__restrict__ x, const int32_t *__restrict__ rowc,
                                                       const int32_t *__restrict__ total, const float *__restrict__ wt,
                                                       const float *__restrict__ bias, float *__restrict__ out, int out_stride, long limit) {
    const long T = *total;
    const int col_tiles = o_dim / 64;
    const long row_tile = bx / col_tiles;
    const int col_tile = (int)(bx - row_tile * col_tiles);
    const long row0 = row_tile * 64;
    if (row0 >= T || (limit >= 0 && T > limit)) return;
    __shared__ float xs[2][GP_KT][GP_XS];
    __shared__ __attribute__((aligned(16))) float ws[2][GP_KT][64];
    const Wave w;
    const int col0 = col_tile * 64;
    const RowsA<1> load_a{{x + min(row0 + (w.tid >> 2), T - 1) * (long)k_dim}, k_dim};
    floatx16 acc[1][1];
    mfma_k_loop<1, 1, false>(w, acc, xs, ws, k_dim, load_a, wt, o_dim, col0);
    const int col = col0 + w.bc;
    int cen[16];
    compact_centres16(rowc, row0 + w.wm * 32 + 16 * w.kh, T, cen);
    compact_pool_atomic(acc[0][0], bias ? bias[col] : 0.f, cen, out + col, out_stride);
}

__global__ __launch_bounds__(256) void gemm_pool_compact_kernel(int k_dim, int o_dim, const float *__restrict__ x, const int32_t *__restrict__ rowc,
                                                                const int32_t *__restrict__ total, const float *__restrict__ wt,
                                                                const float *__restrict__ bias, float *__restrict__ out, int out_stride, long limit) {
    gemm_pool_compact_body(blockIdx.x, k_dim, o_dim, x, rowc, total, wt, bias, out, out_stride, limit);
}

__global__ __launch_bounds__(256) void gemm_pool_compact_pair_kernel(const CompactMlpArgs a0, const CompactMlpArgs a1, const unsigned split, const unsigned total_x) {
    for (unsigned bx = blockIdx.x; bx < total_x; bx += gridDim.x) {
        const bool second = bx >= split;
        const CompactMlpArgs &a = second ? a1 : a0;
        gemm_pool_compact_body(second ? bx - split : bx, a.o2, a.o3, a.mid, a.rowc, a.total, a.w3t, a.b3, a.out, a.out_stride, a.limit);
        __syncthreads();
    }
}

template <int NB1>
__device__ __forceinline__ void pgather_gemm3_compact_body(const unsigned bx, int o2, int o3, int n, int m, const float *__restrict__ pmat, int p_stride,
                                                           const float *__restrict__ xyz, const float *__restrict__ new_xyz,
                                                           const int32_t *__restrict__ rowc, const int32_t *__restrict__ rowsrc,
                                                           const int32_t *__restrict__ total, const float *__restrict__ w1x,
                                                           const float *__restrict__ b1, int relu1, const float *__restrict__ w2t,
                                                           const float *__restrict__ b2, int relu2, const float *__restrict__ w3t,
                                                           const float *__restrict__ b3, float *__restrict__ out, int out_stride, long limit) {
    constexpr int O1 = NB1 * 64;
    const long T = *total;
    const long row0 = (long)bx * 64;
    if (row0 >= T || (limit >= 0 && T > limit)) return;
    extern __shared__ __attribute__((aligned(16))) float smem2[];
    const int o2p = (o2 + GP_KT - 1) / GP_KT * GP_KT;
    float *act = smem2, *act2 = smem2 + O1 * GP_XS, *w2s = smem2 + (O1 + o2p) * GP_XS;
    const Wave w;
    int cidx[16];
    compact_centres16(rowc, row0 + w.wm * 32 + 16 * w.kh, T, cidx);
    ppoint_layer1<NB1>(w, CompactSrc{rowc, rowsrc, row0, T, m}, n, pmat, p_stride, xyz, new_xyz, w1x, b1, relu1, act);
    lds_layer<1>(w, act, O1 / GP_KT, w2t, O1, o2, w2s, 0, 1, [&](const floatx16 &acc, int col) __attribute__((always_inline)) {
        if (col < o2p) store_act(w, acc, b2, relu2, act2, col, o2);
    });
    lds_layer<2>(w, act2, o2p / GP_KT, w3t, o2, o3, smem2, 0, 1, [&](const floatx16 &acc, int col) __attribute__((always_inline)) {
        compact_pool_atomic(acc, b3 ? b3[col] : 0.f, cidx, out + col, out_stride);
    });
}

template <int NB1>
__global__ __launch_bounds__(256) void pgather_gemm3_compact_kernel(int o2, int o3, int n, int m, const float *__restrict__ pmat, int p_stride,
                                                                    const float *__restrict__ xyz, const float *__restrict__ new_xyz,
                                                                    const int32_t *__restrict__ rowc, const int32_t *__restrict__ rowsrc,
                                                                    const int32_t *__restrict__ total, const float *__restrict__ w1x,
                                                                    const float *__restrict__ b1, int relu1, const float *__restrict__ w2t,
                                                                    const float *__restrict__ b2, int relu2, const float *__restrict__ w3t,
                                                                    const float *__restrict__ b3, float *__restrict__ out, int out_stride, long limit) {
    pgather_gemm3_compact_body<NB1>(blockIdx.x, o2, o3, n, m, pmat, p_stride, xyz, new_xyz, rowc, rowsrc, total, w1x, b1, relu1, w2t, b2, relu2, w3t, b3, out,
                                    out_stride, limit);
}

template <int NB1>
__global__ __launch_bounds__(256) void pgather_gemm3_compact_pair_kernel(const CompactMlpArgs a0, const CompactMlpArgs a1, const unsigned split, const unsigned total_x) {
    const bool second = blockIdx.x >= split;
    const CompactMlpArgs &a = second ? a1 : a0;
    pgather_gemm3_compact_body<NB1>(second ? blockIdx.x - split : blockIdx.x, a.o2, a.o3, a.n, a.m, a.pmat, a.p_stride, a.xyz, a.new_xyz, a.rowc, a.rowsrc, a.total,
                                    a.w1x, a.b1, a.relu1, a.w2t, a.b2, a.relu2, a.w3t, a.b3, a.out, a.out_stride, a.limit);
}

__device__ __forceinline__ float4 interp3(float w0, const float4 p0, float w1, const float4 p1, float w2, const float4 p2) {
    return make_float4(__builtin_fmaf(w2, p2.x, __builtin_fmaf(w0, p0.x, w1 * p1.x)), __builtin_fmaf(w2, p2.y, __builtin_fmaf(w0, p0.y, w1 * p1.y)),
                       __builtin_fmaf(w2, p2.z, __builtin_fmaf(w0, p0.z, w1 * p1.z)), __builtin_fmaf(w2, p2.w, __builtin_fmaf(w0, p0.w, w1 * p1.w)));
}
__device__ __forceinline__ float4 ld4(const float *p) { return *reinterpret_cast<const float4 *>(p); }
__device__ __forceinline__ void add4(float4 &y, const float4 a) { y.x += a.x; y.y += a.y; y.z += a.z; y.w += a.w; }
__device__ __forceinline__ void fma4(float4 &y, float s, const float4 a) {
    y.x = __builtin_fmaf(s, a.x, y.x); y.y = __builtin_fmaf(s, a.y, y.y); y.z = __builtin_fmaf(s, a.z, y.z); y.w = __builtin_fmaf(s, a.w, y.w);
}
__device__ __forceinline__ void relu4(float4 &y) { y.x = y.x < 0.f ? 0.f : y.x; y.y = y.y < 0.f ? 0.f : y.y; y.z = y.z < 0.f ? 0.f : y.z; y.w = y.w < 0.f ? 0.f : y.w; }

__device__ __forceinline__ float4 qrow_f4(int k, int o, const float *q0, const float *q1, const float *q2, float w0, float w1, float w2,
                                          const float *lrow, const float *srow, int c1, const float *__restrict__ wb, const float *__restrict__ bias, int relu) {
    float4 y = interp3(w0, ld4(q0 + k), w1, ld4(q1 + k), w2, ld4(q2 + k));
    if (lrow) {
        add4(y, ld4(lrow + k));
    } else {
        for (int j = 0; j < c1; ++j) fma4(y, srow[j], ld4(wb + (long)j * o + k));
        if (bias) add4(y, ld4(bias + k));
    }
    if (relu) relu4(y);
    return y;
}

__global__ __launch_bounds__(256) void qinterp_rows_kernel(long rows, int o, int n, int m, const float *__restrict__ q, const int32_t *__restrict__ idx3,
                                                           const float *__restrict__ w3, const float *__restrict__ lin,
                                                           const float *__restrict__ skip, int c1, const float *__restrict__ wb,
                                                           const float *__restrict__ bias, int relu, float *__restrict__ out) {
    const int q4 = o >> 2;
    const long total = rows * q4;
    for (long e = (long)blockIdx.x * 256 + threadIdx.x; e < total; e += (long)gridDim.x * 256) {
        const long r = e / q4;
        const int c4 = (int)(e - r * q4) * 4;
        const float *qb = q + (size_t)(r / n) * m * o;
        *reinterpret_cast<float4 *>(out + r * (long)o + c4) =
            qrow_f4(c4, o, qb + (size_t)idx3[r * 3 + 0] * o, qb + (size_t)idx3[r * 3 + 1] * o, qb + (size_t)idx3[r * 3 + 2] * o, w3[r * 3 + 0], w3[r * 3 + 1],
                    w3[r * 3 + 2], lin ? lin + r * (long)o : nullptr, skip + r * (long)c1, c1, wb, bias, relu);
    }
}

template <int MB, bool PRE>
struct InterpA {
    const float *f0[MB], *f1[MB], *f2[MB], *urow[MB], *lrow[MB];
    float w0[MB], w1[MB], w2[MB];
    int c2, c1, relu_a;
    const float *wb, *b1;
    __device__ __forceinline__ InterpA(long r0, int c2_, int c1_, int n, int m, const float *__restrict__ known_feats, const float *__restrict__ unknown_feats,
                                       const int32_t *__restrict__ idx3, const float *__restrict__ w3, const float *__restrict__ lin,
                                       const float *__restrict__ wb_, const float *__restrict__ b1_, int relu_a_)
        : c2(c2_), c1(c1_), relu_a(relu_a_), wb(wb_), b1(b1_) {
#pragma unroll
        for (int i = 0; i < MB; ++i) {
            const long r = r0 + 64 * i;
            const float *base = known_feats + (size_t)(r / n) * m * c2;
            f0[i] = base + (size_t)idx3[r * 3 + 0] * c2; f1[i] = base + (size_t)idx3[r * 3 + 1] * c2; f2[i] = base + (size_t)idx3[r * 3 + 2] * c2;
            w0[i] = w3[r * 3 + 0]; w1[i] = w3[r * 3 + 1]; w2[i] = w3[r * 3 + 2];
            urow[i] = unknown_feats ? unknown_feats + (size_t)r * c1 : nullptr;
            lrow[i] = (PRE && lin) ? lin + (size_t)r * c2 : nullptr;
        }
    }
    __device__ __forceinline__ float4 operator()(int i, int k) const {
        if (k < c2) {
            if (PRE) return qrow_f4(k, c2, f0[i], f1[i], f2[i], w0[i], w1[i], w2[i], lrow[i], urow[i], c1, wb, b1, relu_a);
            return interp3(w0[i], ld4(f0[i] + k), w1[i], ld4(f1[i] + k), w2[i], ld4(f2[i] + k));
        }
        if (PRE) return f4_zero();
        const int ku = k - c2;
        if (ku + 3 < c1) return ld4(urow[i] + ku);
        float v[4] = {0.f, 0.f, 0.f, 0.f};
#pragma unroll
        for (int q = 0; q < 4; ++q) if (ku + q < c1) v[q] = urow[i][ku + q];
        return make_float4(v[0], v[1], v[2], v[3]);
    }
};

template <int MB, int NB, bool PRE>
__device__ __forceinline__ void interp_gemm_tile(long vb, float (&xs)[2][GP_KT][64 * MB + 1], float (&ws)[2][GP_KT][64 * NB], int c2, int c1, int o_dim, int n, int m, const float *__restrict__ known_feats,
                                                 const float *__restrict__ unknown_feats, const int32_t *__restrict__ idx3, const float *__restrict__ w3,
                                                 const float *__restrict__ wt, const float *__restrict__ bias, int relu, float *__restrict__ out, int tps,
                                                 const float *__restrict__ lin, const float *__restrict__ wb, const float *__restrict__ b1, int relu_a) {
    const Wave w;
    long row_tile;
    int col_tile;
    gg_tile<true>(o_dim / (64 * NB), tps, vb, row_tile, col_tile);
    const long row0 = row_tile * (64 * MB);
    const int col0 = col_tile * (64 * NB);
    const InterpA<MB, PRE> load_a(row0 + (w.tid >> 2), c2, c1, n, m, known_feats, unknown_feats, idx3, w3, lin, wb, b1, relu_a);
    floatx16 acc[MB][NB];
    mfma_k_loop<MB, NB, false>(w, acc, xs, ws, PRE ? c2 : c2 + c1, load_a, wt, o_dim, col0);
#pragma unroll
    for (int i = 0; i < MB; ++i)
#pragma unroll
        for (int j = 0; j < NB; ++j) store_rows(w, acc[i][j], bias, relu, out, o_dim, row0 + sub_row<MB>(w, i), col0 + sub_col<NB, false>(w, j) + w.l32);
}

__global__ __launch_bounds__(256, 8) void interp_gemm_kernel(int c2, int c1, int o_dim, int n, int m, const float *__restrict__ known_feats,
                                                          const float *__restrict__ unknown_feats, const int32_t *__restrict__ idx3,
                                                          const float *__restrict__ w3, const float *__restrict__ wt,
                                                          const float *__restrict__ bias, int relu, float *__restrict__ out, int tps) {
    __shared__ float xs[2][GP_KT][GP_XS];
    __shared__ __attribute__((aligned(16))) float ws[2][GP_KT][64];
    interp_gemm_tile<1, 1, false>(blockIdx.x, xs, ws, c2, c1, o_dim, n, m, known_feats, unknown_feats, idx3, w3, wt, bias, relu, out, tps, nullptr, nullptr,
                                  nullptr, 0);
}

template <int MB, int NB, bool PRE = false>
__global__ __launch_bounds__(256) void interp_gemm_big_kernel(int c2, int c1, int o_dim, int n, int m, const float *__restrict__ known_feats,
                                                              const float *__restrict__ unknown_feats, const int32_t *__restrict__ idx3,
                                                              const float *__restrict__ w3, const float *__restrict__ wt,
                                                              const float *__restrict__ bias, int relu, float *__restrict__ out, int tps,
                                                              const float *__restrict__ lin = nullptr, const float *__restrict__ wb = nullptr,
                                                              const float *__restrict__ b1 = nullptr, int relu_a = 0, long total_tiles = 0) {
    __shared__ float xs[2][GP_KT][64 * MB + 1];
    __shared__ __attribute__((aligned(16))) float ws[2][GP_KT][64 * NB];
    const long n_tiles = total_tiles > 0 ? total_tiles : (long)gridDim.x;
    for (long vb = blockIdx.x; vb < n_tiles; vb += gridDim.x)
        interp_gemm_tile<MB, NB, PRE>(vb, xs, ws, c2, c1, o_dim, n, m, known_feats, unknown_feats, idx3, w3, wt, bias, relu, out, tps, lin, wb, b1, relu_a);
}

}

extern "C" int ws3d_gemm_pool(long rows, int nsample, int k_dim, int o_dim, const float *x_rows, const float *wt,
                              const float *bias, int relu, float *out, int out_stride, const int32_t *gate, long gate_limit, ws3d_stream_t stream) {
    using namespace ws3d;
    const uintptr_t al = reinterpret_cast<uintptr_t>(x_rows) | reinterpret_cast<uintptr_t>(wt);
    if (rows < 0 || (nsample != 16 && nsample != 32) || k_dim <= 0 || (k_dim & 3) || o_dim <= 0 || (o_dim & 63) || (rows & 63) ||
        !x_rows || !wt || !out || out_stride < o_dim || (al & 15)) {
        set_error("ws3d_gemm_pool: unsupported shape (rows=%ld ns=%d k=%d o=%d; rows, o %% 64, k %% 4, ns 16|32)", rows, nsample,
                  k_dim, o_dim);
        return WS3D_E_UNSUPPORTED;
    }
    if (rows == 0) return WS3D_OK;
    const int mb = (rows % 128 == 0 && o_dim % 128 == 0 && (rows / 128) * (o_dim / 128) >= 512) ? 2 : 1;
    const long row_tiles = rows / (64 * mb);
    const int xcd = row_tiles % 8 == 0 ? 1 : 0;
    const dim3 grid((unsigned)((o_dim / (64 * mb)) * row_tiles)), block(256);
    const auto kern = mb == 2 ? (nsample == 16 ? gemm_pool_big_kernel<16, 2, 2> : gemm_pool_big_kernel<32, 2, 2>)
                              : (nsample == 16 ? gemm_pool_big_kernel<16, 1, 1> : gemm_pool_big_kernel<32, 1, 1>);
    hipLaunchKernelGGL(kern, grid, block, 0, as_stream(stream), k_dim, o_dim, x_rows, wt, bias, relu, out, out_stride, xcd, gate, gate_limit);
    return check_launch("ws3d_gemm_pool");
}

extern "C" int ws3d_gather_gemm(int b, int n, int m, int nsample, int c_feat, int o_dim, const float *feats, const float *xyz,
                                const float *new_xyz, const int32_t *nbr, const float *wt, const float *bias, int relu, float *out,
                                ws3d_stream_t stream) {
    using namespace ws3d;
    const long rows = (long)b * m * nsample;
    const uintptr_t al = reinterpret_cast<uintptr_t>(feats) | reinterpret_cast<uintptr_t>(wt);
    if (b < 0 || n <= 0 || m <= 0 || nsample <= 0 || c_feat <= 0 || (c_feat & 3) || o_dim <= 0 || (o_dim & 63) || (rows & 63) || !feats || !xyz ||
        !new_xyz || !nbr || !wt || !out || (al & 15)) {
        set_error("ws3d_gather_gemm: unsupported shape (b=%d n=%d m=%d ns=%d c=%d o=%d; rows, o %% 64, c %% 4)", b, n, m, nsample, c_feat, o_dim);
        return WS3D_E_UNSUPPORTED;
    }
    if (rows == 0) return WS3D_OK;
    constexpr int xcd_env = 1;
    const long per_scene = (long)m * nsample;
    const int tps = (xcd_env && (b & 7) == 0 && per_scene % 64 == 0) ? (int)(per_scene / 64) : 0;
    hipLaunchKernelGGL(gather_gemm_kernel, dim3((unsigned)((o_dim / 64) * (rows / 64))), dim3(256), 0, as_stream(stream), c_feat, o_dim, n, m,
                       nsample, feats, xyz, new_xyz, nbr, wt, bias, relu, out, tps);
    return check_launch("ws3d_gather_gemm");
}

extern "C" int ws3d_interp_gemm(int b, int n, int m, int c2, int c1, int o_dim, const float *known_feats, const float *unknown_feats,
                                const int32_t *idx, const float *weight, const float *wt, const float *bias, int relu, float *out,
                                ws3d_stream_t stream) {
    using namespace ws3d;
    const long rows = (long)b * n;
    const uintptr_t al = reinterpret_cast<uintptr_t>(known_feats) | reinterpret_cast<uintptr_t>(wt) |
                         ((c1 & 3) == 0 ? reinterpret_cast<uintptr_t>(unknown_feats) : 0);
    if (b < 0 || n <= 0 || m <= 0 || c2 <= 0 || (c2 & 3) || c1 < 0 || o_dim <= 0 || (o_dim & 63) || (rows & 63) || !known_feats ||
        (c1 > 0 && !unknown_feats) || !idx || !weight || !wt || !out || (al & 15)) {
        set_error("ws3d_interp_gemm: unsupported shape (b=%d n=%d m=%d c2=%d c1=%d o=%d; rows, o %% 64, c2 %% 4)", b, n, m, c2, c1, o_dim);
        return WS3D_E_UNSUPPORTED;
    }
    if (rows == 0) return WS3D_OK;
    constexpr int xcd_env = 1;
// ... 274 lines not shown
```

### ws3d_amd/csrc/gemm_rows.hip

```cpp
#include "common.h"
#include "split_bf16.h"

namespace ws3d {

typedef unsigned rows_u4 __attribute__((ext_vector_type(4)));
typedef float rows_f4 __attribute__((ext_vector_type(4)));

constexpr int GR_THREADS = 256;
constexpr int GR_TM = 64;
constexpr int GR_KB = 32;
constexpr int GR_FRAG = 1024;
#ifndef WS3D_GR_TALL_MIN_TILES
#define WS3D_GR_TALL_MIN_TILES 512
#endif
constexpr int GR_TALL_MIN_TILES = WS3D_GR_TALL_MIN_TILES;
constexpr int GR_MAX_DIM = 4096;
__host__ __device__ constexpr int gr_tile_rows(int nbt, int mbw) { return nbt == 4 ? 32 * mbw : 64 * mbw; }
__host__ __device__ constexpr int gr_a_stage(int tm) { return tm / 32 * 2 * 3 * GR_FRAG; }
__host__ __device__ constexpr int gr_lds_bytes(int tm) { return 2 * gr_a_stage(tm); }
static_assert(gr_lds_bytes(128) <= 64 * 1024 && gr_lds_bytes(128) * 2 <= 160 * 1024, "inside the default per-workgroup cap, two workgroups per CU");

__global__ __launch_bounds__(256) void gemm_rows_pack_kernel(int K, int N, const float *__restrict__ wt, rows_u4 *__restrict__ pack) {
    const int nb_all = N / 32;
    const long total = (long)(K / GR_KB) * nb_all * 2 * 64;
    for (long i = (long)blockIdx.x * blockDim.x + threadIdx.x; i < total; i += (long)gridDim.x * blockDim.x) {
        const int lane = (int)(i & 63), s = (int)((i >> 6) & 1);
        const long f = i >> 7;
        const int nb = (int)(f % nb_all), kb = (int)(f / nb_all);
        const int col = nb * 32 + (lane & 31), k0 = kb * GR_KB + 16 * s + 8 * (lane >> 5);
        float v[8];
#pragma unroll
        for (int j = 0; j < 8; ++j) v[j] = wt[(long)(k0 + j) * N + col];
        bf16x8 q1, q2, q3;
        split8(v, q1, q2, q3);
        rows_u4 *dst = pack + ((f * 2 + s) * 3) * 64 + lane;
        dst[0] = __builtin_bit_cast(rows_u4, q1);
        dst[64] = __builtin_bit_cast(rows_u4, q2);
        dst[128] = __builtin_bit_cast(rows_u4, q3);
    }
}

template <int NBT, int MBW>
__global__ __launch_bounds__(GR_THREADS, 2) void gemm_rows_kernel(int K, int N, int ntn, const float *__restrict__ a, const rows_u4 *__restrict__ pack,
                                                                  const float *__restrict__ bias, int relu, float *__restrict__ out) {
    extern __shared__ __attribute__((aligned(16))) unsigned char smem_rows[];
    constexpr int TM = gr_tile_rows(NBT, MBW);
    constexpr int UNITS = TM / 64;
    constexpr int STAGE = gr_a_stage(TM);
    const int tid = threadIdx.x, w = tid >> 6, lane = tid & 63, r = lane & 31, h = lane >> 5;
    const int tn = (int)(blockIdx.x % (unsigned)ntn);
    const long tm = blockIdx.x / (unsigned)ntn;
    const int nb_all = N / 32, nkb = K / GR_KB;
    const int nbl = NBT == 4 ? w : (w & 1), mb0 = NBT == 4 ? 0 : (w >> 1) * MBW;

    const int srow = (lane & 7) + 8 * (lane >> 5) + 16 * w, skq = (lane >> 3) & 3;
    const rows_f4 *ap = reinterpret_cast<const rows_f4 *>(a + (tm * TM + srow) * (long)K + 8 * skq);
    const size_t a_unit = (size_t)16 * K;
    const int a_wr = ((srow >> 5) * 2 + (skq >> 1)) * 3 * GR_FRAG + ((skq & 1) * 32 + (srow & 31)) * 16;
    const rows_u4 *wp = pack + (size_t)(tn * NBT + nbl) * 6 * 64 + lane;
    const size_t w_kb = (size_t)nb_all * 6 * 64;

    floatx16 acc[MBW];
#pragma unroll
    for (int m = 0; m < MBW; ++m)
#pragma unroll
        for (int i = 0; i < 16; ++i) acc[m][i] = 0.f;
    rows_u4 wc[6];
#pragma unroll
    for (int i = 0; i < 6; ++i) wc[i] = rows_u4{0u, 0u, 0u, 0u};

    for (int kb = -1; kb < nkb; ++kb) {
        const bool more = kb + 1 < nkb;
        rows_f4 ra[UNITS][2];
        rows_u4 wn[6];
        if (more) {
#pragma unroll
            for (int u = 0; u < UNITS; ++u) {
                ra[u][0] = ap[u * a_unit + (kb + 1) * (GR_KB / 4)];
                ra[u][1] = ap[u * a_unit + (kb + 1) * (GR_KB / 4) + 1];
            }
#pragma unroll
            for (int i = 0; i < 6; ++i) wn[i] = wp[(kb + 1) * w_kb + i * 64];
        }
        if (kb >= 0) {
            const unsigned char *buf = smem_rows + (kb & 1) * STAGE + lane * 16;
#pragma unroll
            for (int s = 0; s < 2; ++s) {
                const bf16x8 w1 = __builtin_bit_cast(bf16x8, wc[3 * s]), w2 = __builtin_bit_cast(bf16x8, wc[3 * s + 1]),
                               w3 = __builtin_bit_cast(bf16x8, wc[3 * s + 2]);
                bf16x8 a1[MBW], a2[MBW], a3[MBW];
#pragma unroll
                for (int m = 0; m < MBW; ++m) {
                    const unsigned char *af = buf + ((mb0 + m) * 2 + s) * 3 * GR_FRAG;
                    a1[m] = *reinterpret_cast<const bf16x8 *>(af);
                    a2[m] = *reinterpret_cast<const bf16x8 *>(af + GR_FRAG);
                    a3[m] = *reinterpret_cast<const bf16x8 *>(af + 2 * GR_FRAG);
                }
                split_mfma6<MBW>(w1, w2, w3, a1, a2, a3, acc);
            }
        }
        if (more) {
            unsigned char *nxt = smem_rows + ((kb + 1) & 1) * STAGE + a_wr;
#pragma unroll
            for (int u = 0; u < UNITS; ++u) {
                const float v[8] = {ra[u][0][0], ra[u][0][1], ra[u][0][2], ra[u][0][3], ra[u][1][0], ra[u][1][1], ra[u][1][2], ra[u][1][3]};
                bf16x8 q1, q2, q3;
                split8(v, q1, q2, q3);
                *reinterpret_cast<bf16x8 *>(nxt + u * 12 * GR_FRAG) = q1;
                *reinterpret_cast<bf16x8 *>(nxt + u * 12 * GR_FRAG + GR_FRAG) = q2;
                *reinterpret_cast<bf16x8 *>(nxt + u * 12 * GR_FRAG + 2 * GR_FRAG) = q3;
            }
#pragma unroll
            for (int i = 0; i < 6; ++i) wc[i] = wn[i];
        }
        __syncthreads();
    }

    const int n0 = (tn * NBT + nbl) * 32 + 4 * h;
    rows_f4 b4[4];
    if (bias) {
#pragma unroll
        for (int g = 0; g < 4; ++g) b4[g] = *reinterpret_cast<const rows_f4 *>(bias + n0 + 8 * g);
    }
#pragma unroll
    for (int m = 0; m < MBW; ++m) {
        float *orow = out + (tm * TM + (mb0 + m) * 32 + r) * (long)N + n0;
#pragma unroll
        for (int g = 0; g < 4; ++g) {
            rows_f4 y;
#pragma unroll
            for (int e = 0; e < 4; ++e) y[e] = acc[m][4 * g + e];
            if (bias) y = y + b4[g];
            if (relu) {
#pragma unroll
                for (int e = 0; e < 4; ++e) y[e] = relu_keep_nan(y[e]);
            }
            *reinterpret_cast<rows_f4 *>(orow + 8 * g) = y;
        }
    }
}

static bool gr_dims_ok(int K, int N) { return K >= GR_KB && K <= GR_MAX_DIM && K % GR_KB == 0 && N >= 64 && N <= GR_MAX_DIM && N % 64 == 0; }

}

extern "C" size_t ws3d_gemm_rows_pack_bytes(int k_dim, int n_dim) {
    return ws3d::gr_dims_ok(k_dim, n_dim) ? (size_t)k_dim * n_dim * 6 : 0;
}

extern "C" int ws3d_gemm_rows_pack(int k_dim, int n_dim, const float *wt, void *pack, ws3d_stream_t stream) {
    using namespace ws3d;
    if (!wt || !pack || (reinterpret_cast<uintptr_t>(pack) & 15) || (reinterpret_cast<uintptr_t>(wt) & 3)) {
        set_error("ws3d_gemm_rows_pack: invalid argument");
        return WS3D_E_INVALID;
    }
    if (!gr_dims_ok(k_dim, n_dim)) {
        set_error("ws3d_gemm_rows_pack: unsupported shape K=%d N=%d (K %% 32, N %% 64, both <= %d)", k_dim, n_dim, GR_MAX_DIM);
        return WS3D_E_UNSUPPORTED;
    }
    const long threads = (long)(k_dim / GR_KB) * (n_dim / 32) * 128;
    hipLaunchKernelGGL(gemm_rows_pack_kernel, dim3((unsigned)((threads + 255) / 256)), dim3(256), 0, as_stream(stream), k_dim, n_dim, wt,
                       static_cast<rows_u4 *>(pack));
    return check_launch("ws3d_gemm_rows_pack");
}

extern "C" int ws3d_gemm_rows_split(long rows, int k_dim, int n_dim, const float *a, const void *pack, const float *bias, int relu, float *out,
                                    ws3d_stream_t stream) {
    using namespace ws3d;
    if (rows < 0 || k_dim <= 0 || n_dim <= 0 || !a || !pack || !out) {
        set_error("ws3d_gemm_rows_split: invalid argument (rows=%ld K=%d N=%d)", rows, k_dim, n_dim);
        return WS3D_E_INVALID;
    }
    const uintptr_t al = reinterpret_cast<uintptr_t>(a) | reinterpret_cast<uintptr_t>(pack) | reinterpret_cast<uintptr_t>(out) | reinterpret_cast<uintptr_t>(bias);
    const int nbt = n_dim % 128 == 0 ? 4 : 2;
    if (!gr_dims_ok(k_dim, n_dim) || rows % GR_TM || (al & 15) || (rows / GR_TM) * (n_dim / (32 * nbt)) > 0x7fffffffL) {
        set_error("ws3d_gemm_rows_split: unsupported shape or alignment (rows=%ld K=%d N=%d; rows %% 64, K %% 32, N %% 64, 16-byte pointers)", rows,
                  k_dim, n_dim);
        return WS3D_E_UNSUPPORTED;
    }
    if (rows == 0) return WS3D_OK;
    const int ntn = n_dim / (32 * nbt);
    const bool tall = nbt == 4 && rows % 128 == 0 && (rows / 128) * ntn >= GR_TALL_MIN_TILES;
    const int tm = tall ? 128 : 64;
    const unsigned grid = (unsigned)((rows / tm) * ntn);
    auto go = [&](auto kern) -> int {
        hipLaunchKernelGGL(kern, dim3(grid), dim3(GR_THREADS), (size_t)gr_lds_bytes(tm), as_stream(stream), k_dim, n_dim, ntn, a,
                           static_cast<const rows_u4 *>(pack), bias, relu ? 1 : 0, out);
        return WS3D_OK;
    };
    if (int rc = nbt == 2 ? go(gemm_rows_kernel<2, 1>) : tall ? go(gemm_rows_kernel<4, 4>) : go(gemm_rows_kernel<4, 2>)) return rc;
    return check_launch("ws3d_gemm_rows_split");
}
```

### ws3d_amd/fastpath.py

```python
from __future__ import annotations

import contextlib
import contextvars

import torch
import torch.nn as nn

from . import compat as _C
from . import nn_blocks, pn2_ops

FUSED_SA_MLP = True
SA1_FROM_LISTS = True
FUSED_GEMM_POOL = True
FUSED_INTERP_GEMM = True
NESTED_FPS = True
GEOMETRY_AHEAD = True
_AHEAD_OVERRIDE = contextvars.ContextVar("ws3d_geometry_ahead", default=None)


@contextlib.contextmanager
def geometry_ahead(on: bool):
    token = _AHEAD_OVERRIDE.set(bool(on))
    try:
        yield
    finally:
        _AHEAD_OVERRIDE.reset(token)


@contextlib.contextmanager
def compact_only_scales(keys):
    token = _COMPACT_ONLY.set(frozenset(keys))
    try:
        yield
    finally:
        _COMPACT_ONLY.reset(token)


def primed_compact_scales(net, pointcloud: torch.Tensor, margin: float = None):
    margin = PRIMED_MARGIN if margin is None else margin
    keys, per_level = set(), {}
    for row in list_fill(net, pointcloud):
        si = per_level.get(row["level"], 0)
        per_level[row["level"]] = si + 1
        if row["fill"] <= margin * COMPACT_MAX_FILL:
            keys.add((row["level"] - 1, si))
    return frozenset(keys)


def _geometry_ahead_now() -> bool:
    v = _AHEAD_OVERRIDE.get()
    return GEOMETRY_AHEAD if v is None else v
GEOMETRY_IN_CAPTURE = False
PER_POINT_L1 = True
COMPACT_MAX_FILL = 0.55
COMPACT_PAIRS = True
PAIR_DISPATCH = "device"
PRIMED_MARGIN = 0.85
_COMPACT_ONLY = contextvars.ContextVar("ws3d_compact_only_scales", default=frozenset())
CHAIN_MLP = True
PAIRED_SCALES = True
MERGED_THREE_NN = True
FUSED_PROLOGUE = True
MERGED_BINNING = True
PER_POINT_FP = True
FUSED_MLP2_ROWS = True
FUSED_HEADS = True
SPLIT_GEMMS = True
FUSED_GATHER_GEMM2 = True
BIN_INPUT_AHEAD = True
FUSED_QINTERP_GEMM_MIN_ROWS = 30000
FUSED_COMPACT3_MAX_LDS = 64 * 1024
FUSED_GATHER_GEMM = True
GRID_MIN_N = 256
DUAL_SCALE_SEARCH = True
NESTED_CHAIN = True
QUERY_CELL_ORDER = True
PARALLEL_SCALES = True
PARALLEL_HEADS = True


def _row_weights(block):
    w, shift, act = block._folded()
    if act is not None and not isinstance(act, nn.ReLU):
        raise NotImplementedError("fast path supports ReLU / no activation only")
    cache = block.__dict__.get("_row_cache")
    if cache is None or cache[0] is not w:
        cache = (w, w.t().contiguous())
        if not torch.cuda.is_current_stream_capturing():
            block.__dict__["_row_cache"] = cache
    return cache[1], shift, act is not None


def _row_weights_xyz_last(block):
    wt, bias, relu = _row_weights(block)
    cache = block.__dict__.get("_row_cache_xyz_last")
    if cache is None or cache[0] is not wt:
        cache = (wt, torch.cat((wt[3:], wt[:3]), dim=0).contiguous())
        if not torch.cuda.is_current_stream_capturing():
            block.__dict__["_row_cache_xyz_last"] = cache
    return cache[1], bias, relu


def _split_rows(block, wt: torch.Tensor, c2: int):
    cache = block.__dict__.get("_split_cache")
    if cache is None or cache[0] is not wt or cache[1] != c2:
        cache = (wt, c2, wt[:c2].contiguous(), wt[c2:].contiguous())
        if not torch.cuda.is_current_stream_capturing():
            block.__dict__["_split_cache"] = cache
    return cache[2], cache[3]


_SPLIT_GEMM_LIBRARY_WINS = frozenset({(512, 1024, 512)})


def _split_gemm_wins(rows: int, k: int, n: int) -> bool:
    return (rows, k, n) not in _SPLIT_GEMM_LIBRARY_WINS


def _split_gemm(x2d: torch.Tensor, holder, key: str, wt: torch.Tensor, bias=None, relu: bool = False):
    if not SPLIT_GEMMS or x2d.dim() != 2 or not _split_gemm_wins(x2d.size(0), wt.size(0), wt.size(1)):
        return None
    packs = holder.__dict__.get("_gemm_rows_packs")
    ent = None if packs is None else packs.get(key)
    if ent is None or ent[0] is not wt:
        if torch.cuda.is_current_stream_capturing():
            return None
        ent = (wt, _C.gemm_rows_pack(wt))
        holder.__dict__.setdefault("_gemm_rows_packs", {})[key] = ent
    if ent[1] is None:
        return None
    return _C.gemm_rows_split(x2d, ent[1], wt.size(1), bias, relu)


def gemm_rows_packs(model):
    return [ent[1] for m in model.modules() for ent in m.__dict__.get("_gemm_rows_packs", {}).values() if ent[1] is not None]


def _layer(x2d: torch.Tensor, block) -> torch.Tensor:
    wt, bias, relu = _row_weights(block)
    y = _split_gemm(x2d, block, "row", wt, bias, relu)
    if y is not None:
        return y
    if bias is None:
        y = torch.mm(x2d, wt)
        return torch.relu_(y) if relu else y
    if relu:
        return torch._addmm_activation(bias, x2d, wt, use_gelu=False)
    return torch.addmm(bias, x2d, wt)


def _blocks(seq):
    return [m for m in seq if isinstance(m, nn_blocks._ConvBlock)]


def mlp_rows(x2d: torch.Tensor, seq, ticket=None) -> torch.Tensor:
    blocks = _blocks(seq)
    if FUSED_MLP2_ROWS and len(blocks) == 2 and x2d.size(1) == 128 and x2d.is_contiguous():
        (w1, b1, r1), (w2, b2, r2) = _row_weights(blocks[0]), _row_weights(blocks[1])
        y = _C.mlp2_rows(x2d, w1, b1, r1, w2, b2, r2, ticket)
        if y is not None:
            return y
    for blk in blocks:
        x2d = _layer(x2d, blk)
    return x2d


def _heads_blob(seq):
    blocks = _blocks(seq)
    if len(blocks) != 2:
        return None
    (w1, b1, r1), (w2, b2, r2) = _row_weights(blocks[0]), _row_weights(blocks[1])
    cache = blocks[0].__dict__.get("_heads_blob")
    if cache is None or cache[0] is not w1 or cache[1] is not b1 or cache[2] is not w2 or cache[3] is not b2:
        cache = (w1, b1, w2, b2, _C.rpn_heads_pack(w1, b1, r1, w2, b2, r2), w2.size(1))
        if not torch.cuda.is_current_stream_capturing():
            blocks[0].__dict__["_heads_blob"] = cache
    return None if cache[4] is None else (cache[4], cache[5])


def heads_blobs(rpn):
    return [blk.__dict__["_heads_blob"][4] for seq in (rpn.rpn_cls_layer, rpn.rpn_reg_layer) for blk in _blocks(seq)[:1]
            if "_heads_blob" in blk.__dict__]


def _fused_heads(rows: torch.Tensor, blobs, which: int, tickets):
    if blobs is None or not all(blobs[i] is not None for i in (0, 1) if which & (1 << i)):
        return None
    (bc, oc), (br, orr) = blobs[0] or (None, 1), blobs[1] or (None, 0)
    if oc != 1 or (which & 2 and orr == 1):
        return None
    return _C.rpn_heads(rows, which, bc, br, orr, tickets, _C.tune("mlp2_wgs") * (2 if which == 3 else 1))


def supported(model) -> bool:
    try:
        for m in model.modules():
            if isinstance(m, nn_blocks._ConvBlock):
                if not m._pointwise or not isinstance(getattr(m, "activation", None), (nn.ReLU, type(None))):
                    return False
        for sa in model.rpn.backbone_net.SA_modules:
            if sa.pool_method != "max_pool" or sa.npoint is None:
                return False
            for g, mlp in zip(sa.groupers, sa.mlps):
                if not isinstance(g, pn2_ops.QueryAndGroup) or any(b.conv.out_channels % 4 for b in _blocks(mlp)):
                    return False
        return True
    except AttributeError:
        return False


def _gather_gemm_ok(sa, grouper, blocks, c_feat: int, B: int) -> bool:
    return (FUSED_GATHER_GEMM and c_feat >= 16 and c_feat % 4 == 0 and grouper.use_xyz and len(blocks) >= 2 and
            blocks[0].conv.out_channels % 64 == 0 and (B * sa.npoint * grouper.nsample) % 64 == 0 and
            (B * sa.npoint * grouper.nsample) // 64 <= 65535)


def _pair_limit(rows: int, dense_available: bool, key=None) -> int:
    if PAIR_DISPATCH != "device" or not dense_available or (key is not None and key in _COMPACT_ONLY.get()):
        return -1
    return max(0, int(COMPACT_MAX_FILL * rows))


@torch.no_grad()
def list_fill(net, pointcloud: torch.Tensor):
    xyz = pointcloud[..., 0:3].contiguous()
    rows = []
    for level, sa in enumerate(net.SA_modules):
        _, new_xyz = (pn2_ops.furthest_point_sample_gather_nested if NESTED_FPS and level >= 1 else pn2_ops.furthest_point_sample_gather)(xyz, sa.npoint)
        srt = pn2_ops.sort_points_x(xyz)
        for g in sa.groupers:
            nbr = _C.ball_query_lists(g.radius, g.nsample, xyz, new_xyz, srt)
            total = _C.compact_pairs(nbr)[2]
            rows.append({"level": level + 1, "n": xyz.size(1), "npoint": sa.npoint, "radius": float(g.radius), "nsample": g.nsample,
                         "distinct_per_list": float(total.item()) / max(nbr.numel() // g.nsample, 1),
                         "fill": float(total.item()) / max(nbr.numel(), 1)})
        xyz = new_xyz
    return rows


class _ZeroArena:

    def __init__(self, numel: int, device, clear: bool = True):
        n = (max(int(numel), 4) + 3) & ~3
        self.buf = (torch.zeros if clear else torch.empty)(n, dtype=torch.float32, device=device)
        self.dirty = not clear
        self.off = 0
        self.fallbacks = 0

    def ensure_clear(self):
        if self.dirty:
            self.buf.zero_()
            self.dirty = False

    def take(self, shape, dtype=torch.float32):
        n = 1
        for d in shape:
            n *= int(d)
        if self.off + n > self.buf.numel():
            self.fallbacks += 1
            self.fallback_shapes = getattr(self, "fallback_shapes", []) + [(tuple(shape), self.off, self.buf.numel())]
            return torch.zeros(shape, dtype=dtype, device=self.buf.device)
        v = self.buf[self.off:self.off + n]
        self.off += (n + 3) & ~3
        return (v if dtype == torch.float32 else v.view(dtype)).view(shape)


LAST_ARENA_FALLBACKS = 0


def _arena_for(net, B: int, device, extra: int = 0, clear: bool = True) -> _ZeroArena:
    n = extra + 64
    if COMPACT_PAIRS:
        for sa in net.SA_modules:
            n += B * sa.npoint * sum(_blocks(mlp)[-1].conv.out_channels for mlp in sa.mlps) + 4
            n += 4 * len(sa.groupers)
        if CHAIN_MLP:
            n += _C.chain_ticket_ints() + 4
    return _ZeroArena(n, device, clear)


class _PairList:
    __slots__ = ("nbr", "pairs")

    def __init__(self, nbr, pairs):
# ... 173 lines not shown
        if nbr is not None:
            wt1, b1, r1 = _row_weights_xyz_last(blocks[0])
            if PER_POINT_L1 and len(blocks) >= 3:
                if pp[0] is None:
                    pp[0] = _per_point_l1(sa, feats, nbrs)
                pmat, offs, w1xs = pp[0]
                o1 = blocks[0].conv.out_channels
                y = None
                wt3, b3, r3 = _row_weights(blocks[-1])
                if pairs is not None and o1 <= 256 and len(blocks) == 3 and r3:
                    wt2, b2, r2 = _row_weights(blocks[1])
                    rows, ns, o3 = nbr.numel(), grouper.nsample, wt3.size(1)
                    dense_ok = (o1 in (64, 128) and (sa.npoint * ns) % 64 == 0 and rows // 64 <= 65535 and o3 % 64 == 0 and
                                wt2.size(1) % 4 == 0 and ns in (16, 32))
                    limit = _pair_limit(rows, dense_ok, (level, si))
                    fused = _C.pgather_gemm3_compact(pmat, offs[si], o1, xyz, new_xyz, pairs, w1xs[si], b1, r1, wt2, b2, r2, wt3, b3, out, col,
                                                     limit=limit, max_lds=FUSED_COMPACT3_MAX_LDS)
                    yc = None if fused else _C.pgather_gemm2_compact(pmat, offs[si], o1, xyz, new_xyz, pairs, w1xs[si], b1, r1, wt2, b2, r2, limit=limit)
                    if fused or (yc is not None and _C.gemm_pool_compact(yc, pairs, wt3, b3, out, col, limit=limit)):
                        if limit >= 0:
                            gate = (pairs[2], limit)
                            yd = _C.pgather_gemm2(pmat, offs[si], o1, xyz, new_xyz, nbr, w1xs[si], b1, r1, wt2, b2, r2, out=yc, gate=gate)
                            if yd is None or not _C.gemm_pool(yd, wt3, b3, r3, ns, out, col, gate=gate):
                                yc = _C.pgather_gemm2_compact(pmat, offs[si], o1, xyz, new_xyz, pairs, w1xs[si], b1, r1, wt2, b2, r2, limit=-1)
                                if yc is None or not _C.gemm_pool_compact(yc, pairs, wt3, b3, out, col, limit=-1):
                                    raise RuntimeError("neither the gated dense nor the ungated compact kernels took the shape")
                        return
                if o1 <= 128:
                    wt2, b2, r2 = _row_weights(blocks[1])
                    y = _C.pgather_gemm2(pmat, offs[si], o1, xyz, new_xyz, nbr, w1xs[si], b1, r1, wt2, b2, r2)
                    rest_pp = blocks[2:-1]
                if y is None:
                    y = _C.pgather_rows(pmat, offs[si], o1, xyz, new_xyz, nbr, w1xs[si], b1, r1)
                    rest_pp = blocks[1:-1]
                if y is not None:
                    for blk in rest_pp:
                        y = _layer(y, blk)
                    wt, bias, relu = _row_weights(blocks[-1])
                    if not (FUSED_GEMM_POOL and _C.gemm_pool(y, wt, bias, relu, grouper.nsample, out, col)):
                        _C.rowmax_rows(_layer(y, blocks[-1]), grouper.nsample, out, col)
                    return
            y = None
            rest = blocks[1:-1]
            if FUSED_GATHER_GEMM2 and len(blocks) >= 3 and blocks[0].conv.out_channels <= 128:
                wt2, b2, r2 = _row_weights(blocks[1])
                y = _C.gather_gemm2(feats, xyz, new_xyz, nbr, wt1, b1, r1, wt2, b2, r2)
                if y is not None:
                    rest = blocks[2:-1]
            if y is None:
                y = _C.gather_gemm(feats, xyz, new_xyz, nbr, wt1, b1, r1)
            if y is not None:
                for blk in rest:
                    y = _layer(y, blk)
                wt, bias, relu = _row_weights(blocks[-1])
                if not (FUSED_GEMM_POOL and _C.gemm_pool(y, wt, bias, relu, grouper.nsample, out, col)):
                    _C.rowmax_rows(_layer(y, blocks[-1]), grouper.nsample, out, col)
                return
        if FUSED_SA_MLP and SA1_FROM_LISTS and feats is not None and feats.size(2) == 1 and grouper.use_xyz and len(blocks) == 3:
            layers = [_row_weights(b) for b in blocks]
            if not COMPACT_PAIRS:
                nbr1 = _C.ball_query_lists(grouper.radius, grouper.nsample, xyz, new_xyz, sorted_xyz)
                if _C.sa_mlp3_pool_lists(xyz, new_xyz, feats, nbr1, layers, out, col):
                    return
            else:
                nbr1, pairs1 = sa1_pairs[si] if si in sa1_pairs else _lists_and_pairs(grouper.radius, grouper.nsample, xyz, new_xyz, sorted_xyz, zeros)
                limit = _pair_limit(nbr1.numel(), layers[2][2] and nbr1.numel() % 32 == 0 and grouper.nsample in (16, 32), (level, si))
                if _C.sa_mlp3_pool_compact(xyz, new_xyz, feats, pairs1, layers, out, col, limit=limit):
                    if limit >= 0 and not _C.sa_mlp3_pool_lists(xyz, new_xyz, feats, nbr1, layers, out, col, gate=(pairs1[2], limit)):
                        if not _C.sa_mlp3_pool_compact(xyz, new_xyz, feats, pairs1, layers, out, col, limit=-1):
                            raise RuntimeError("neither ws3d_sa_mlp3_pool_lists nor the ungated compact kernel took the shape")
                    return
        g = _C.query_and_group_nlc(grouper.radius, grouper.nsample, xyz, new_xyz, feats, grouper.use_xyz, sorted_xyz)
        rows = g.view(-1, g.size(3))
        if not (FUSED_SA_MLP and rows.size(1) == 4 and len(blocks) == 3 and
                _C.sa_mlp3_pool(rows, grouper.nsample, [_row_weights(b) for b in blocks], out, col)):
            y = rows
            for blk in blocks[:-1]:
                y = _layer(y, blk)
            wt, bias, relu = _row_weights(blocks[-1])
            if not (FUSED_GEMM_POOL and _C.gemm_pool(y, wt, bias, relu, grouper.nsample, out, col)):
                _C.rowmax_rows(_layer(y, blocks[-1]), grouper.nsample, out, col)

    def run_paired() -> bool:
        if not (PAIRED_SCALES and COMPACT_PAIRS and PER_POINT_L1 and len(widths) == 2 and all(isinstance(n_, _PairList) for n_ in nbrs)):
            return False
        blk = [_blocks(m_) for m_ in sa.mlps]
        if any(len(b_) != 3 or b_[0].conv.out_channels > 256 for b_ in blk) or blk[0][0].conv.out_channels != blk[1][0].conv.out_channels:
            return False
        if any(_pair_limit(n_.nbr.numel(), True, (level, si_)) != -1 for si_, n_ in enumerate(nbrs)):
            return False
        if pp[0] is None:
            pp[0] = _per_point_l1(sa, feats, nbrs)
        pmat, offs, w1xs = pp[0]
        scales = []
        for si_ in range(2):
            _w1, b1, r1 = _row_weights_xyz_last(blk[si_][0])
            wt2, b2, r2 = _row_weights(blk[si_][1])
            wt3, b3, r3 = _row_weights(blk[si_][2])
            if not r3:
                return False
            scales.append({"pmat": pmat, "col0": offs[si_], "o1": blk[si_][0].conv.out_channels, "xyz": xyz, "new_xyz": new_xyz, "pairs": nbrs[si_].pairs,
                           "w1x": w1xs[si_], "b1": b1, "relu1": r1, "w2t": wt2, "b2": b2, "relu2": r2, "w3t": wt3, "b3": b3, "out2d": out, "col_offset": cols[si_]})
        if (CHAIN_MLP and zeros is not None and all(sc_["o1"] == 64 and sc_["w2t"].size(1) <= 96 and sc_["w3t"].size(1) == 128 for sc_ in scales)
                and _C.chain_mlp3(scales, zeros.take((_C.chain_ticket_ints(),), torch.int32))):
            return True
        if _C.compact_mlp_pair(3, scales, max_lds=FUSED_COMPACT3_MAX_LDS):
            return True
        mids = _C.compact_mlp_pair(2, scales)
        if mids is None:
            return False
        if not _C.compact_mlp_pair(1, scales, mids=mids):
            for sc_, mid in zip(scales, mids):
                if not _C.gemm_pool_compact(mid, sc_["pairs"], sc_["w3t"], sc_["b3"], out, sc_["col_offset"], limit=-1):
                    raise RuntimeError("ws3d_gemm_pool_compact declined a shape ws3d_pgather_gemm2_compact took")
        return True

    if run_paired():
        pass
    elif geo is not None and geo.aux is not None and PARALLEL_SCALES and len(widths) == 2:
        if PER_POINT_L1 and any(n is not None and len(_blocks(m)) >= 3 for n, m in zip(nbrs, sa.mlps)):
            pp[0] = _per_point_l1(sa, feats, nbrs)
        fork = torch.cuda.Event()
        fork.record(geo.main)
        geo.aux.wait_event(fork)
        with torch.cuda.stream(geo.aux):
            run_scale(1)
            join = torch.cuda.Event()
            join.record(geo.aux)
        run_scale(0)
        geo.main.wait_event(join)
    else:
        for si in range(len(widths)):
            run_scale(si)
    return new_xyz, out.view(B, sa.npoint, -1)


def fp_forward(fp, unknown: torch.Tensor, known: torch.Tensor, unknown_feats, known_feats: torch.Tensor, nn3=None, sorted_unknown=None,
               known_xz=None):
    B, n = unknown.size(0), unknown.size(1)
    idx, weight = nn3 if nn3 is not None else _C.three_nn_with_weights(unknown, known, known_xz[0] if known_xz is not None else pn2_ops.sort_points_xz(known),
                                                                        sorted_unknown if QUERY_CELL_ORDER else None)
    c2 = known_feats.size(2)
    c1 = 0 if unknown_feats is None else unknown_feats.size(2)
    blocks = _blocks(fp.mlp)
    if PER_POINT_FP and blocks and blocks[0].conv.out_channels % 4 == 0:
        wt1, b1, r1 = _row_weights(blocks[0])
        wa, wb = _split_rows(blocks[0], wt1, c2)
        m = known_feats.size(1)
        q = _split_gemm(known_feats.reshape(B * m, c2), blocks[0], "wa", wa)
        q = (q if q is not None else torch.mm(known_feats.reshape(B * m, c2), wa)).view(B, m, -1)
        fuse2 = len(blocks) == 2 and B * n >= FUSED_QINTERP_GEMM_MIN_ROWS
        if fuse2:
            wt2, b2, r2 = _row_weights(blocks[1])
        if c1 > 4:
            lin = _split_gemm(unknown_feats.reshape(B * n, c1), blocks[0], "wb", wb, b1)
            if lin is None:
                lin = torch.mm(unknown_feats.reshape(B * n, c1), wb) if b1 is None else torch.addmm(b1, unknown_feats.reshape(B * n, c1), wb)
            y = _C.qinterp_gemm(q, idx, weight, wt2, b2, r2, lin=lin, relu=r1) if fuse2 else None
            if y is not None:
                return y.view(B, n, -1)
            y = _C.qinterp_rows(q, idx, weight, lin=lin, relu=r1)
        else:
            sk = None if c1 == 0 else unknown_feats.contiguous()
            y = _C.qinterp_gemm(q, idx, weight, wt2, b2, r2, skip=sk, wb=wb if c1 else None, bias=b1, relu=r1) if fuse2 else None
            if y is not None:
                return y.view(B, n, -1)
            y = _C.qinterp_rows(q, idx, weight, skip=sk, wb=wb if c1 else None, bias=b1, relu=r1)
        if y is not None:
            for blk in blocks[1:]:
                y = _layer(y, blk)
            return y.view(B, n, -1)
    if FUSED_INTERP_GEMM and blocks and blocks[0].conv.out_channels % 64 == 0 and B * n >= 8192:
        wt1, b1, r1 = _row_weights(blocks[0])
        y = _C.interp_gemm(known_feats.contiguous(), None if unknown_feats is None else unknown_feats.contiguous(), idx, weight, wt1, b1, r1)
        if y is not None:
            for blk in blocks[1:]:
                y = _layer(y, blk)
            return y.view(B, n, -1)
    cat = torch.empty((B, n, c2 + c1), dtype=torch.float32, device=unknown.device)
    _C.three_interpolate_nlc(known_feats, idx, weight, cat)
    if c1:
        cat[:, :, c2:] = unknown_feats
    return mlp_rows(cat.view(B * n, c2 + c1), fp.mlp).view(B, n, -1)


@torch.no_grad()
def backbone_forward(net, pointcloud: torch.Tensor, zeros: _ZeroArena = None):
    if FUSED_PROLOGUE and pointcloud.is_cuda and pointcloud.dim() == 3 and pointcloud.is_contiguous() and pointcloud.size(-1) > 3:
        if zeros is None:
            zeros = _arena_for(net, pointcloud.size(0), pointcloud.device, clear=False)
        xyz, feats = _C.split_points_clear(pointcloud, zeros.buf if zeros.dirty else None)
        zeros.dirty = False
    else:
        xyz = pointcloud[..., 0:3].contiguous()
        feats = pointcloud[..., 3:].contiguous() if pointcloud.size(-1) > 3 else None
        if zeros is None:
            zeros = _arena_for(net, xyz.size(0), xyz.device)
        zeros.ensure_clear()
    ahead = _geometry_ahead_now() and (GEOMETRY_IN_CAPTURE or not torch.cuda.is_current_stream_capturing())
    geo = _Geometry(net, xyz, 0 if feats is None else feats.size(2), zeros) if ahead else None
    l_xyz, l_feats, binned = [xyz], [feats], []
    try:
        sas, chain, pre_grid, pre_xz, nn_pre = list(net.SA_modules), None, {}, {}, {}
        for level, sa in enumerate(sas):
            pre = chain[level - 1][1] if (chain is not None and level >= 1) else None
            nx, nf = sa_forward(sa, l_xyz[-1], l_feats[-1], geo, level, zeros, binned, pre, pre_grid.get(level))
            l_xyz.append(nx)
            l_feats.append(nf)
            if geo is None and level == 0 and NESTED_FPS and NESTED_CHAIN and len(sas) > 1:
                chain = pn2_ops.furthest_point_sample_gather_nested_chain(nx, [s_.npoint for s_ in sas[1:]])
                if MERGED_BINNING:
                    lv = [nx] + [c[1] for c in chain]
                    jobs = [(x_, "grid") for x_ in lv[:-1] if x_.size(1) >= GRID_MIN_N] + [(x_, "xz") for x_ in lv if x_.size(1) >= 256]
                    bufs = iter(_C.sort_points_jobs(jobs) if _C.BQ_FINE_GRID else [])
                    if _C.BQ_FINE_GRID:
                        pre_grid = {k + 1: ((next(bufs),) if x_.size(1) >= GRID_MIN_N else (None,)) for k, x_ in enumerate(lv[:-1])}
                        pre_xz = {k + 1: (next(bufs) if x_.size(1) >= 256 else None) for k, x_ in enumerate(lv)}
                        if MERGED_THREE_NN:
                            allx = [l_xyz[0]] + lv
                            qgrid = {0: binned[0]}
                            qgrid.update({k_: v_[0] for k_, v_ in pre_grid.items()})
                            lvls = [k_ for k_ in range(len(sas)) if pre_xz.get(k_ + 1) is not None and allx[k_ + 1].size(1) <= 4096]
                            got = _C.three_nn_jobs([(allx[k_], allx[k_ + 1], pre_xz[k_ + 1], qgrid.get(k_) if QUERY_CELL_ORDER else None) for k_ in lvls])
                            if got is not None:
                                nn_pre = dict(zip(lvls, got))
        for i in range(-1, -(len(net.FP_modules) + 1), -1):
            lvl = len(l_xyz) + i - 1
            nn3 = nn_pre.get(lvl)
            if geo is not None:
                geo.main.wait_event(geo.nn_ready[lvl])
                nn3 = geo.nn[lvl]
            known_level = len(l_xyz) + i
            l_feats[i - 1] = fp_forward(net.FP_modules[i], l_xyz[i - 1], l_xyz[i], l_feats[i - 1], l_feats[i], nn3, binned[len(l_xyz) + i - 1],
                                        (pre_xz[known_level],) if known_level in pre_xz else None)
    finally:
        if geo is not None:
            geo.release()
    return l_xyz[0], l_feats[0]


@torch.no_grad()
def rpn_forward(model, pts_input: torch.Tensor, defer_reg_join: bool = False) -> dict:
    rpn = model.rpn
    zeros = _arena_for(rpn.backbone_net, pts_input.size(0), pts_input.device, extra=8, clear=not FUSED_PROLOGUE)
    xyz, feats = backbone_forward(rpn.backbone_net, pts_input, zeros)
    B, N, C = feats.shape
    rows = feats.view(B * N, C)
    tickets = zeros.take((2,), torch.int32) if (FUSED_MLP2_ROWS or FUSED_HEADS) else (None, None)
    blobs = (_heads_blob(rpn.rpn_cls_layer), _heads_blob(rpn.rpn_reg_layer)) if FUSED_HEADS else None
    reg_ready = None
    if PARALLEL_HEADS and _geometry_ahead_now() and not torch.cuda.is_current_stream_capturing():
        main = torch.cuda.current_stream(rows.device)
        aux = _side_streams(main)[2]
        fork = torch.cuda.Event()
        fork.record(main)
        aux.wait_event(fork)
        with torch.cuda.stream(aux):
            fused = _fused_heads(rows, blobs, 2, tickets)
            rpn_reg = (fused[1] if fused is not None else mlp_rows(rows, rpn.rpn_reg_layer, tickets[1:2])).view(B, N, -1)
            reg_ready = torch.cuda.Event()
            reg_ready.record(aux)
        rpn_reg.record_stream(main)
        fused = _fused_heads(rows, blobs, 1, tickets)
        rpn_cls = (fused[0] if fused is not None else mlp_rows(rows, rpn.rpn_cls_layer, tickets[0:1])).view(B, N, -1)
        if not defer_reg_join:
            main.wait_event(reg_ready)
            reg_ready = None
    else:
        fused = _fused_heads(rows, blobs, 3, tickets)
        if fused is not None:
            rpn_cls, rpn_reg = fused[0].view(B, N, -1), fused[1].view(B, N, -1)
        else:
            rpn_cls = mlp_rows(rows, rpn.rpn_cls_layer, tickets[0:1]).view(B, N, -1)
            rpn_reg = mlp_rows(rows, rpn.rpn_reg_layer, tickets[1:2]).view(B, N, -1)
    global LAST_ARENA_FALLBACKS
    LAST_ARENA_FALLBACKS = zeros.fallbacks if not zeros.fallbacks else getattr(zeros, "fallback_shapes", zeros.fallbacks)
    out = {"rpn_cls": rpn_cls, "rpn_reg": rpn_reg, "backbone_xyz": xyz,
           "backbone_features": feats.transpose(1, 2),
           "backbone_features_nlc": feats}
    if reg_ready is not None:
        out["rpn_reg_ready"] = reg_ready
    return out
```

Baseline: 7084.

## Fuse three-point interpolation into split-bf16 MFMA row GEMM for FP layers

Adds a new kernel that computes the interpolated FP first-layer activations (3-NN weighted gather plus lin or skip term, bias, ReLU) directly inside the A-operand producer of the split-bf16 MFMA row GEMM, and uses it for the second FP layer. The gemm_rows kernel body is refactored into a shared header templated on the A source so both paths reuse it. Small skip weights and bias are optionally staged in LDS. This replaces the previous fused qinterp_gemm path when a weight pack is available, aiming to use matrix cores instead of the older fused kernel. The trade-off is reduced precision from the bf16 split and extra gather loads per K block.

```diff
diff --git a/include/ws3d_ops.h b/include/ws3d_ops.h
--- a/include/ws3d_ops.h
+++ b/include/ws3d_ops.h
@@ -241,6 +241,10 @@
                       const float *skip, int c1, const float *wb, const float *b1, int relu1, const float *w2t, const float *b2, int relu2,
                       float *out, ws3d_stream_t stream);
 
+WS3D_API int ws3d_qinterp_gemm_split(int b, int n, int m, int c, int o_dim, const float *q, const int32_t *idx, const float *weight, const float *lin,
+                            const float *skip, int c1, const float *wb, const float *b1, int relu1, const void *pack, const float *b2, int relu2,
+                            float *out, ws3d_stream_t stream);
+
 
 WS3D_API int ws3d_boxes_overlap_bev(int num_a, const float *boxes_a, int num_b, const float *boxes_b,
                            float *ans, ws3d_stream_t stream);
diff --git a/ws3d_amd/_lib.py b/ws3d_amd/_lib.py
--- a/ws3d_amd/_lib.py
+++ b/ws3d_amd/_lib.py
@@ -70,6 +70,7 @@
     "ws3d_rowmax_rows": (_i, [C.c_long, _i, _i, _vp, _vp, _i, _vp]),
     "ws3d_sa_mlp3_pool": (_i, [C.c_long, _i, _i, _i, _i, _vp, _vp, _vp, _vp, _vp, _vp, _vp, _i, _vp, _i, _vp]),
     "ws3d_qinterp_gemm": (_i, [_i, _i, _i, _i, _i, _vp, _vp, _vp, _vp, _vp, _i, _vp, _vp, _i, _vp, _vp, _i, _vp, _vp]),
+    "ws3d_qinterp_gemm_split": (_i, [_i, _i, _i, _i, _i, _vp, _vp, _vp, _vp, _vp, _i, _vp, _vp, _i, _vp, _vp, _i, _vp, _vp]),
     "ws3d_mlp2_rows": (_i, [C.c_long, _i, _i, _i, _vp, _vp, _vp, _i, _vp, _vp, _i, _vp, _vp, _vp]),
     "ws3d_rpn_heads_blob_bytes": (_sz, [_i]),
     "ws3d_rpn_heads_pack": (_i, [_i, _vp, _vp, _i, _vp, _vp, _i, _vp, _vp]),
diff --git a/ws3d_amd/build.py b/ws3d_amd/build.py
--- a/ws3d_amd/build.py
+++ b/ws3d_amd/build.py
@@ -18,7 +18,7 @@
 def lib_path(dist_mode: int = 0) -> str:
     return LIB if dist_mode == 0 else os.path.join(HERE, "libws3d_hip_dm%d.so" % dist_mode)
 ARCH = "gfx950"
-SOURCES = ["core.hip", "fps.hip", "fps_v3.hip", "fps_bucket.hip", "fps_nested.hip", "fps_ragged.hip", "fps_pruned.hip", "ballquery_group.hip", "interpolate.hip", "roipool3d.hip", "iou3d.hip", "proposals.hip", "scatter_det.hip", "sa_mlp.hip", "bn_relu.hip", "gemm_pool.hip", "conv_wgrad.hip", "chain_mlp.hip", "rpn_heads.hip", "gemm_rows.hip", "kitti_eval.hip", "instance_clouds.hip", "click.hip", "stage2.hip", "stage2_ragged.hip", "stage2_loss.hip", "rpn_targets.hip", "scan_prepare.hip", "stage2_batch.hip"]
+SOURCES = ["core.hip", "fps.hip", "fps_v3.hip", "fps_bucket.hip", "fps_nested.hip", "fps_ragged.hip", "fps_pruned.hip", "ballquery_group.hip", "interpolate.hip", "roipool3d.hip", "iou3d.hip", "proposals.hip", "scatter_det.hip", "sa_mlp.hip", "bn_relu.hip", "gemm_pool.hip", "conv_wgrad.hip", "chain_mlp.hip", "rpn_heads.hip", "gemm_rows.hip", "fp_split.hip", "kitti_eval.hip", "instance_clouds.hip", "click.hip", "stage2.hip", "stage2_ragged.hip", "stage2_loss.hip", "rpn_targets.hip", "scan_prepare.hip", "stage2_batch.hip"]
 CXXFLAGS = ["-O3", "-std=c++17", "-fPIC", "-ffp-contract=off", "-fno-fast-math",
             "-fvisibility=hidden", "-Wall", "-Wno-unused-function"]
 
diff --git a/ws3d_amd/compat.py b/ws3d_amd/compat.py
--- a/ws3d_amd/compat.py
+++ b/ws3d_amd/compat.py
@@ -564,7 +564,9 @@
     return out
 
 
-def qinterp_gemm(q, idx, weight, w2t, b2, relu2, lin=None, skip=None, wb=None, bias=None, relu=True):
+def qinterp_gemm(q, idx, weight, w2t, b2, relu2, lin=None, skip=None, wb=None, bias=None, relu=True, pack=None):
+    if pack is not None:
+        return _qinterp_gemm_split(q, idx, weight, w2t, pack, b2, relu2, lin, skip, wb, bias, relu)
     dev = _dev(q, idx, weight, w2t)
     _f32(q, "q"); _i32(idx, "idx"); _f32(weight, "weight"); _f32(w2t, "w2t")
     B, M, C = q.shape
@@ -579,6 +581,34 @@
     with _on(dev):
         check(_lib.load().ws3d_qinterp_gemm(B, N, M, C, O, _p(q), _p(idx), _p(weight), _p(lin), _p(skip), c1, _p(wb), _p(bias), int(bool(relu)), _p(w2t),
                                             _p(b2), int(bool(relu2)), _p(out), _stream()), "qinterp_gemm")
+    return out
+
+
+def _qinterp_gemm_split(q, idx, weight, w2t, pack, b2, relu2, lin, skip, wb, bias, relu):
+    dev = _dev(q, idx, weight, w2t, pack)
+    _f32(q, "q"); _i32(idx, "idx"); _f32(weight, "weight"); _f32(w2t, "w2t")
+    B, M, C = q.shape
+    N = idx.size(1)
+    O = w2t.size(1)
+    c1 = 0 if skip is None else skip.size(2)
+    if ((B * N) % 64 or C % 32 or O % 64 or w2t.size(0) != C or pack.numel() * pack.element_size() < C * O * 6 or not q.is_contiguous() or
+            not idx.is_contiguous() or not weight.is_contiguous() or (b2 is not None and (not b2.is_contiguous() or b2.numel() != O)) or
+            (lin is None and c1 > 4) or (lin is not None and (tuple(lin.shape) != (B * N, C) or not lin.is_contiguous())) or
+            (lin is None and c1 > 0 and (wb is None or tuple(wb.shape) != (c1, C) or not wb.is_contiguous() or not skip.is_contiguous())) or
+            (lin is None and bias is not None and (not bias.is_contiguous() or bias.numel() != C))):
+        return None
+    for t, name in ((lin, "lin"), (skip, "skip"), (wb, "wb"), (bias, "bias"), (b2, "b2")):
+        if t is not None:
+            _f32(t, name)
+    if any(t is not None and t.data_ptr() % 16 for t in (q, pack, lin, wb, bias, b2)):
+        return None
+    out = torch.empty((B * N, O), dtype=torch.float32, device=dev)
+    with _on(dev):
+        rc = _lib.load().ws3d_qinterp_gemm_split(B, N, M, C, O, _p(q), _p(idx), _p(weight), _p(lin), _p(skip), c1, _p(wb), _p(bias), int(bool(relu)),
+                                                 _p(pack), _p(b2), int(bool(relu2)), _p(out), _stream())
+    if rc == _lib.E_UNSUPPORTED:
+        return None
+    check(rc, "qinterp_gemm_split")
     return out
 
 
diff --git a/ws3d_amd/csrc/fp_split.hip b/ws3d_amd/csrc/fp_split.hip
--- /dev/null
+++ b/ws3d_amd/csrc/fp_split.hip
@@ -0,0 +1,119 @@
+#include "gemm_rows_core.h"
+#include "mfma_tile.h"
+#include "qinterp_row.h"
+
+namespace ws3d {
+
+template <int UNITS>
+struct FpRowsA {
+    static constexpr int RAW = 8;
+    static __device__ __forceinline__ int srow(int tid) { return (tid >> 2) & 63; }
+    static __device__ __forceinline__ int skq(int tid) { return tid & 3; }
+    const float *q0[UNITS], *q1[UNITS], *q2[UNITS], *xrow[UNITS];
+    float w0[UNITS], w1[UNITS], w2[UNITS];
+    const float *wb, *b1;
+    int c, c1, k0, relu1;
+    bool has_lin;
+    __device__ __forceinline__ FpRowsA(long row0, int skq, int c_, int c1_, int n, int m, const float *__restrict__ q, const int32_t *__restrict__ idx3,
+                                       const float *__restrict__ w3, const float *__restrict__ lin, const float *skip, long skip_row0,
+                                       const float *wb_, const float *b1_, int relu1_)
+        : wb(wb_), b1(b1_), c(c_), c1(c1_), k0(8 * skq), relu1(relu1_), has_lin(lin != nullptr) {
+#pragma unroll
+        for (int u = 0; u < UNITS; ++u) {
+            const long r = row0 + 64 * u;
+            const float *base = q + (size_t)(r / n) * m * c + k0;
+            q0[u] = base + (size_t)idx3[r * 3 + 0] * c; q1[u] = base + (size_t)idx3[r * 3 + 1] * c; q2[u] = base + (size_t)idx3[r * 3 + 2] * c;
+            w0[u] = w3[r * 3 + 0]; w1[u] = w3[r * 3 + 1]; w2[u] = w3[r * 3 + 2];
+            xrow[u] = lin ? lin + (size_t)r * c + k0 : skip + (size_t)(r - skip_row0) * c1;
+        }
+    }
+    __device__ __forceinline__ void fetch(int kb, rows_f4 (&ra)[UNITS][RAW]) const {
+        const int k = kb * GR_KB;
+#pragma unroll
+        for (int u = 0; u < UNITS; ++u) {
+#pragma unroll
+            for (int e = 0; e < 2; ++e) {
+                ra[u][e] = *reinterpret_cast<const rows_f4 *>(q0[u] + k + 4 * e);
+                ra[u][2 + e] = *reinterpret_cast<const rows_f4 *>(q1[u] + k + 4 * e);
+                ra[u][4 + e] = *reinterpret_cast<const rows_f4 *>(q2[u] + k + 4 * e);
+                if (has_lin) ra[u][6 + e] = *reinterpret_cast<const rows_f4 *>(xrow[u] + k + 4 * e);
+            }
+        }
+    }
+    __device__ __forceinline__ void values(int u, int kb, const rows_f4 (&ra)[UNITS][RAW], float (&v)[8]) const {
+        const auto f4 = [](const rows_f4 x) { return make_float4(x[0], x[1], x[2], x[3]); };
+#pragma unroll
+        for (int e = 0; e < 2; ++e) {
+            const float4 y = qrow_f4_of(kb * GR_KB + k0 + 4 * e, c, f4(ra[u][e]), f4(ra[u][2 + e]), f4(ra[u][4 + e]), w0[u], w1[u], w2[u], has_lin,
+                                        has_lin ? f4(ra[u][6 + e]) : make_float4(0.f, 0.f, 0.f, 0.f), xrow[u], c1, wb, b1, relu1);
+            v[4 * e] = y.x; v[4 * e + 1] = y.y; v[4 * e + 2] = y.z; v[4 * e + 3] = y.w;
+        }
+    }
+};
+
+constexpr int FP_STAGE_MAX = 16 * 1024;
+__host__ __device__ constexpr int fp_stage_floats(int tm, int c, int c1, bool has_b1) { return (c1 + (has_b1 ? 1 : 0)) * c + tm * c1; }
+
+template <int NBT, int MBW, bool STAGED>
+__global__ __launch_bounds__(GR_THREADS, 2) void fp_split_kernel(int c, int o_dim, int ntn, int tps, int n, int m, const float *__restrict__ q,
+                                                                 const int32_t *__restrict__ idx3, const float *__restrict__ w3, const float *__restrict__ lin,
+                                                                 const float *__restrict__ skip, int c1, const float *__restrict__ wb,
+                                                                 const float *__restrict__ b1, int relu1, const rows_u4 *__restrict__ pack,
+                                                                 const float *__restrict__ b2, int relu2, float *__restrict__ out) {
+    extern __shared__ __attribute__((aligned(16))) unsigned char smem_fp[];
+    constexpr int TM = gr_tile_rows(NBT, MBW);
+    long tm;
+    int tn;
+    if (tps > 0) gg_tile<true>(ntn, tps, blockIdx.x, tm, tn); else gg_tile<false>(ntn, -tps, blockIdx.x, tm, tn);
+    using Src = FpRowsA<TM / 64>;
+    if (STAGED) {
+        float *cst = reinterpret_cast<float *>(smem_fp + gr_lds_bytes(TM));
+        float *cb1 = cst + c1 * c, *csk = cb1 + (b1 ? c : 0);
+        for (int i = threadIdx.x; i < c1 * c; i += GR_THREADS) cst[i] = wb[i];
+        if (b1)
+            for (int i = threadIdx.x; i < c; i += GR_THREADS) cb1[i] = b1[i];
+        for (int i = threadIdx.x; i < TM * c1; i += GR_THREADS) csk[i] = skip[tm * TM * c1 + i];
+        __syncthreads();
+        const Src src(tm * TM + Src::srow(threadIdx.x), Src::skq(threadIdx.x), c, c1, n, m, q, idx3, w3, nullptr, csk, tm * TM, cst, b1 ? cb1 : nullptr, relu1);
+        gr_tile<NBT, MBW>(smem_fp, c, o_dim, tm, tn, src, pack, b2, relu2, out);
+        return;
+    }
+    const Src src(tm * TM + Src::srow(threadIdx.x), Src::skq(threadIdx.x), c, c1, n, m, q, idx3, w3, lin, skip, 0, wb, b1, relu1);
+    gr_tile<NBT, MBW>(smem_fp, c, o_dim, tm, tn, src, pack, b2, relu2, out);
+}
+
+}
+
+extern "C" int ws3d_qinterp_gemm_split(int b, int n, int m, int c, int o_dim, const float *q, const int32_t *idx, const float *weight, const float *lin,
+                                      const float *skip, int c1, const float *wb, const float *b1, int relu1, const void *pack, const float *b2, int relu2,
+                                      float *out, ws3d_stream_t stream) {
+    using namespace ws3d;
+    const long rows = (long)b * n;
+    const uintptr_t al = reinterpret_cast<uintptr_t>(q) | reinterpret_cast<uintptr_t>(pack) | reinterpret_cast<uintptr_t>(lin) | reinterpret_cast<uintptr_t>(wb) |
+                         reinterpret_cast<uintptr_t>(b1) | reinterpret_cast<uintptr_t>(b2) | reinterpret_cast<uintptr_t>(out);
+    const uintptr_t al4 = reinterpret_cast<uintptr_t>(idx) | reinterpret_cast<uintptr_t>(weight) | reinterpret_cast<uintptr_t>(skip);
+    const int nbt = o_dim % 128 == 0 ? 4 : 2;
+    if (b < 0 || n <= 0 || m <= 0 || c <= 0 || o_dim <= 0 || !gr_dims_ok(c, o_dim) || (rows % GR_TM) || !q || !idx || !weight || !pack || !out || (al & 15) ||
+        (al4 & 3) || (!lin && (c1 < 0 || c1 > 4 || (c1 > 0 && (!skip || !wb)))) || (rows / GR_TM) * (o_dim / (32 * nbt)) > 0x7fffffffL) {
+        set_error("ws3d_qinterp_gemm_split: unsupported shape or alignment (b=%d n=%d m=%d c=%d o=%d c1=%d; rows %% 64, c %% 32, o %% 64, 16-byte pointers, lin or c1 <= 4)",
+                  b, n, m, c, o_dim, c1);
+        return WS3D_E_UNSUPPORTED;
+    }
+    if (rows == 0) return WS3D_OK;
+    const int ntn = o_dim / (32 * nbt);
+    constexpr int tm = GR_TM;
+    const int tps = (b % 8 == 0 && n % tm == 0) ? n / tm : ((rows / tm) % 8 == 0 ? -1 : 0);
+    const unsigned grid = (unsigned)((rows / tm) * ntn);
+    const int stage = (!lin && (c1 > 0 || b1)) ? 4 * fp_stage_floats(tm, c, c1, b1 != nullptr) : 0;
+    const bool staged = stage > 0 && stage <= FP_STAGE_MAX;
+    auto go = [&](auto kern) {
+        hipLaunchKernelGGL(kern, dim3(grid), dim3(GR_THREADS), (size_t)gr_lds_bytes(tm) + (staged ? stage : 0), as_stream(stream), c, o_dim, ntn, tps, n, m, q, idx, weight, lin,
+                           lin ? nullptr : skip, lin ? 0 : c1, wb, b1, relu1 ? 1 : 0, static_cast<const rows_u4 *>(pack), b2, relu2 ? 1 : 0, out);
+    };
+    if (staged) {
+        if (nbt == 2) go(fp_split_kernel<2, 1, true>); else go(fp_split_kernel<4, 2, true>);
+    } else {
+        if (nbt == 2) go(fp_split_kernel<2, 1, false>); else go(fp_split_kernel<4, 2, false>);
+    }
+    return check_launch("ws3d_qinterp_gemm_split");
+}
diff --git a/ws3d_amd/csrc/gemm_pool.hip b/ws3d_amd/csrc/gemm_pool.hip
--- a/ws3d_amd/csrc/gemm_pool.hip
+++ b/ws3d_amd/csrc/gemm_pool.hip
@@ -3,6 +3,7 @@
 #include "common.h"
 #include "compact_pool.h"
 #include "mfma_tile.h"
+#include "qinterp_row.h"
 
 namespace ws3d {
 
@@ -339,29 +340,6 @@
                                     a.w1x, a.b1, a.relu1, a.w2t, a.b2, a.relu2, a.w3t, a.b3, a.out, a.out_stride, a.limit);
 }
 
-__device__ __forceinline__ float4 interp3(float w0, const float4 p0, float w1, const float4 p1, float w2, const float4 p2) {
-    return make_float4(__builtin_fmaf(w2, p2.x, __builtin_fmaf(w0, p0.x, w1 * p1.x)), __builtin_fmaf(w2, p2.y, __builtin_fmaf(w0, p0.y, w1 * p1.y)),
-                       __builtin_fmaf(w2, p2.z, __builtin_fmaf(w0, p0.z, w1 * p1.z)), __builtin_fmaf(w2, p2.w, __builtin_fmaf(w0, p0.w, w1 * p1.w)));
-}
-__device__ __forceinline__ float4 ld4(const float *p) { return *reinterpret_cast<const float4 *>(p); }
-__device__ __forceinline__ void add4(float4 &y, const float4 a) { y.x += a.x; y.y += a.y; y.z += a.z; y.w += a.w; }
-__device__ __forceinline__ void fma4(float4 &y, float s, const float4 a) {
-    y.x = __builtin_fmaf(s, a.x, y.x); y.y = __builtin_fmaf(s, a.y, y.y); y.z = __builtin_fmaf(s, a.z, y.z); y.w = __builtin_fmaf(s, a.w, y.w);
-}
-__device__ __forceinline__ void relu4(float4 &y) { y.x = y.x < 0.f ? 0.f : y.x; y.y = y.y < 0.f ? 0.f : y.y; y.z = y.z < 0.f ? 0.f : y.z; y.w = y.w < 0.f ? 0.f : y.w; }
-
-__device__ __forceinline__ float4 qrow_f4(int k, int o, const float *q0, const float *q1, const float *q2, float w0, float w1, float w2,
-                                          const float *lrow, const float *srow, int c1, const float *__restrict__ wb, const float *__restrict__ bias, int relu) {
-    float4 y = interp3(w0, ld4(q0 + k), w1, ld4(q1 + k), w2, ld4(q2 + k));
-    if (lrow) {
-        add4(y, ld4(lrow + k));
-    } else {
-        for (int j = 0; j < c1; ++j) fma4(y, srow[j], ld4(wb + (long)j * o + k));
-        if (bias) add4(y, ld4(bias + k));
-    }
-    if (relu) relu4(y);
-    return y;
-}
 
 __global__ __launch_bounds__(256) void qinterp_rows_kernel(long rows, int o, int n, int m, const float *__restrict__ q, const int32_t *__restrict__ idx3,
                                                            const float *__restrict__ w3, const float *__restrict__ lin,
diff --git a/ws3d_amd/csrc/gemm_rows.hip b/ws3d_amd/csrc/gemm_rows.hip
--- a/ws3d_amd/csrc/gemm_rows.hip
+++ b/ws3d_amd/csrc/gemm_rows.hip
@@ -1,24 +1,6 @@
-#include "common.h"
-#include "split_bf16.h"
+#include "gemm_rows_core.h"
 
 namespace ws3d {
-
-typedef unsigned rows_u4 __attribute__((ext_vector_type(4)));
-typedef float rows_f4 __attribute__((ext_vector_type(4)));
-
-constexpr int GR_THREADS = 256;
-constexpr int GR_TM = 64;
-constexpr int GR_KB = 32;
-constexpr int GR_FRAG = 1024;
-#ifndef WS3D_GR_TALL_MIN_TILES
-#define WS3D_GR_TALL_MIN_TILES 512
-#endif
-constexpr int GR_TALL_MIN_TILES = WS3D_GR_TALL_MIN_TILES;
-constexpr int GR_MAX_DIM = 4096;
-__host__ __device__ constexpr int gr_tile_rows(int nbt, int mbw) { return nbt == 4 ? 32 * mbw : 64 * mbw; }
-__host__ __device__ constexpr int gr_a_stage(int tm) { return tm / 32 * 2 * 3 * GR_FRAG; }
-__host__ __device__ constexpr int gr_lds_bytes(int tm) { return 2 * gr_a_stage(tm); }
-static_assert(gr_lds_bytes(128) <= 64 * 1024 && gr_lds_bytes(128) * 2 <= 160 * 1024, "inside the default per-workgroup cap, two workgroups per CU");
 
 __global__ __launch_bounds__(256) void gemm_rows_pack_kernel(int K, int N, const float *__restrict__ wt, rows_u4 *__restrict__ pack) {
     const int nb_all = N / 32;
@@ -45,102 +27,12 @@
                                                                   const float *__restrict__ bias, int relu, float *__restrict__ out) {
     extern __shared__ __attribute__((aligned(16))) unsigned char smem_rows[];
     constexpr int TM = gr_tile_rows(NBT, MBW);
-    constexpr int UNITS = TM / 64;
-    constexpr int STAGE = gr_a_stage(TM);
-    const int tid = threadIdx.x, w = tid >> 6, lane = tid & 63, r = lane & 31, h = lane >> 5;
     const int tn = (int)(blockIdx.x % (unsigned)ntn);
     const long tm = blockIdx.x / (unsigned)ntn;
-    const int nb_all = N / 32, nkb = K / GR_KB;
-    const int nbl = NBT == 4 ? w : (w & 1), mb0 = NBT == 4 ? 0 : (w >> 1) * MBW;
-
-    const int srow = (lane & 7) + 8 * (lane >> 5) + 16 * w, skq = (lane >> 3) & 3;
-    const rows_f4 *ap = reinterpret_cast<const rows_f4 *>(a + (tm * TM + srow) * (long)K + 8 * skq);
-    const size_t a_unit = (size_t)16 * K;
-    const int a_wr = ((srow >> 5) * 2 + (skq >> 1)) * 3 * GR_FRAG + ((skq & 1) * 32 + (srow & 31)) * 16;
-    const rows_u4 *wp = pack + (size_t)(tn * NBT + nbl) * 6 * 64 + lane;
-    const size_t w_kb = (size_t)nb_all * 6 * 64;
-
-    floatx16 acc[MBW];
-#pragma unroll
-    for (int m = 0; m < MBW; ++m)
-#pragma unroll
-        for (int i = 0; i < 16; ++i) acc[m][i] = 0.f;
-    rows_u4 wc[6];
-#pragma unroll
-    for (int i = 0; i < 6; ++i) wc[i] = rows_u4{0u, 0u, 0u, 0u};
-
-    for (int kb = -1; kb < nkb; ++kb) {
-        const bool more = kb + 1 < nkb;
-        rows_f4 ra[UNITS][2];
-        rows_u4 wn[6];
-        if (more) {
-#pragma unroll
-            for (int u = 0; u < UNITS; ++u) {
-                ra[u][0] = ap[u * a_unit + (kb + 1) * (GR_KB / 4)];
-                ra[u][1] = ap[u * a_unit + (kb + 1) * (GR_KB / 4) + 1];
-            }
-#pragma unroll
-            for (int i = 0; i < 6; ++i) wn[i] = wp[(kb + 1) * w_kb + i * 64];
-        }
-        if (kb >= 0) {
-            const unsigned char *buf = smem_rows + (kb & 1) * STAGE + lane * 16;
-#pragma unroll
-            for (int s = 0; s < 2; ++s) {
-                const bf16x8 w1 = __builtin_bit_cast(bf16x8, wc[3 * s]), w2 = __builtin_bit_cast(bf16x8, wc[3 * s + 1]),
-                               w3 = __builtin_bit_cast(bf16x8, wc[3 * s + 2]);
-                bf16x8 a1[MBW], a2[MBW], a3[MBW];
-#pragma unroll
-                for (int m = 0; m < MBW; ++m) {
-                    const unsigned char *af = buf + ((mb0 + m) * 2 + s) * 3 * GR_FRAG;
-                    a1[m] = *reinterpret_cast<const bf16x8 *>(af);
-                    a2[m] = *reinterpret_cast<const bf16x8 *>(af + GR_FRAG);
-                    a3[m] = *reinterpret_cast<const bf16x8 *>(af + 2 * GR_FRAG);
-                }
-                split_mfma6<MBW>(w1, w2, w3, a1, a2, a3, acc);
-            }
-        }
-        if (more) {
-            unsigned char *nxt = smem_rows + ((kb + 1) & 1) * STAGE + a_wr;
-#pragma unroll
-            for (int u = 0; u < UNITS; ++u) {
-                const float v[8] = {ra[u][0][0], ra[u][0][1], ra[u][0][2], ra[u][0][3], ra[u][1][0], ra[u][1][1], ra[u][1][2], ra[u][1][3]};
-                bf16x8 q1, q2, q3;
-                split8(v, q1, q2, q3);
-                *reinterpret_cast<bf16x8 *>(nxt + u * 12 * GR_FRAG) = q1;
-                *reinterpret_cast<bf16x8 *>(nxt + u * 12 * GR_FRAG + GR_FRAG) = q2;
-                *reinterpret_cast<bf16x8 *>(nxt + u * 12 * GR_FRAG + 2 * GR_FRAG) = q3;
-            }
-#pragma unroll
-            for (int i = 0; i < 6; ++i) wc[i] = wn[i];
-        }
-        __syncthreads();
-    }
-
-    const int n0 = (tn * NBT + nbl) * 32 + 4 * h;
-    rows_f4 b4[4];
-    if (bias) {
-#pragma unroll
-        for (int g = 0; g < 4; ++g) b4[g] = *reinterpret_cast<const rows_f4 *>(bias + n0 + 8 * g);
-    }
-#pragma unroll
-    for (int m = 0; m < MBW; ++m) {
-        float *orow = out + (tm * TM + (mb0 + m) * 32 + r) * (long)N + n0;
-#pragma unroll
-        for (int g = 0; g < 4; ++g) {
-            rows_f4 y;
-#pragma unroll
-            for (int e = 0; e < 4; ++e) y[e] = acc[m][4 * g + e];
-            if (bias) y = y + b4[g];
-            if (relu) {
-#pragma unroll
-                for (int e = 0; e < 4; ++e) y[e] = relu_keep_nan(y[e]);
-            }
-            *reinterpret_cast<rows_f4 *>(orow + 8 * g) = y;
-        }
-    }
+    using Src = GrRowsA<TM / 64>;
+    const Src src(a, tm * TM + Src::srow(threadIdx.x), K, Src::skq(threadIdx.x));
+    gr_tile<NBT, MBW>(smem_rows, K, N, tm, tn, src, pack, bias, relu, out);
 }
-
-static bool gr_dims_ok(int K, int N) { return K >= GR_KB && K <= GR_MAX_DIM && K % GR_KB == 0 && N >= 64 && N <= GR_MAX_DIM && N % 64 == 0; }
 
 }
 
diff --git a/ws3d_amd/csrc/gemm_rows_core.h b/ws3d_amd/csrc/gemm_rows_core.h
--- /dev/null
+++ b/ws3d_amd/csrc/gemm_rows_core.h
@@ -0,0 +1,143 @@
+#pragma once
+#include "common.h"
+#include "split_bf16.h"
+
+namespace ws3d {
+
+typedef unsigned rows_u4 __attribute__((ext_vector_type(4)));
+typedef float rows_f4 __attribute__((ext_vector_type(4)));
+
+constexpr int GR_THREADS = 256;
+constexpr int GR_TM = 64;
+constexpr int GR_KB = 32;
+constexpr int GR_FRAG = 1024;
+#ifndef WS3D_GR_TALL_MIN_TILES
+#define WS3D_GR_TALL_MIN_TILES 512
+#endif
+constexpr int GR_TALL_MIN_TILES = WS3D_GR_TALL_MIN_TILES;
+constexpr int GR_MAX_DIM = 4096;
+__host__ __device__ constexpr int gr_tile_rows(int nbt, int mbw) { return nbt == 4 ? 32 * mbw : 64 * mbw; }
+__host__ __device__ constexpr int gr_a_stage(int tm) { return tm / 32 * 2 * 3 * GR_FRAG; }
+__host__ __device__ constexpr int gr_lds_bytes(int tm) { return 2 * gr_a_stage(tm); }
+static_assert(gr_lds_bytes(128) <= 64 * 1024 && gr_lds_bytes(128) * 2 <= 160 * 1024, "inside the default per-workgroup cap, two workgroups per CU");
+
+static inline bool gr_dims_ok(int K, int N) { return K >= GR_KB && K <= GR_MAX_DIM && K % GR_KB == 0 && N >= 64 && N <= GR_MAX_DIM && N % 64 == 0; }
+
+template <int UNITS>
+struct GrRowsA {
+    static constexpr int RAW = 2;
+    static __device__ __forceinline__ int srow(int tid) {
+        const int w = tid >> 6, lane = tid & 63;
+        return (lane & 7) + 8 * (lane >> 5) + 16 * w;
+    }
+    static __device__ __forceinline__ int skq(int tid) { return ((tid & 63) >> 3) & 3; }
+    const rows_f4 *ap;
+    size_t a_unit;
+    __device__ __forceinline__ GrRowsA(const float *__restrict__ a, long row0, int K, int skq)
+        : ap(reinterpret_cast<const rows_f4 *>(a + row0 * (long)K + 8 * skq)), a_unit((size_t)16 * K) {}
+    __device__ __forceinline__ void fetch(int kb, rows_f4 (&ra)[UNITS][RAW]) const {
+#pragma unroll
+        for (int u = 0; u < UNITS; ++u) {
+            ra[u][0] = ap[u * a_unit + kb * (GR_KB / 4)];
+            ra[u][1] = ap[u * a_unit + kb * (GR_KB / 4) + 1];
+        }
+    }
+    __device__ __forceinline__ void values(int u, int, const rows_f4 (&ra)[UNITS][RAW], float (&v)[8]) const {
+#pragma unroll
+        for (int e = 0; e < 4; ++e) { v[e] = ra[u][0][e]; v[4 + e] = ra[u][1][e]; }
+    }
+};
+
+template <int NBT, int MBW, class ASrc>
+__device__ __forceinline__ void gr_tile(unsigned char *smem_rows, int K, int N, long tm, int tn, const ASrc src, const rows_u4 *__restrict__ pack,
+                                        const float *__restrict__ bias, int relu, float *__restrict__ out) {
+    constexpr int TM = gr_tile_rows(NBT, MBW);
+    constexpr int UNITS = TM / 64;
+    constexpr int STAGE = gr_a_stage(TM);
+    const int tid = threadIdx.x, w = tid >> 6, lane = tid & 63, r = lane & 31, h = lane >> 5;
+    const int nb_all = N / 32, nkb = K / GR_KB;
+    const int nbl = NBT == 4 ? w : (w & 1), mb0 = NBT == 4 ? 0 : (w >> 1) * MBW;
+
+    const int srow = ASrc::srow(tid), skq = ASrc::skq(tid);
+    const int a_wr = ((srow >> 5) * 2 + (skq >> 1)) * 3 * GR_FRAG + ((skq & 1) * 32 + (srow & 31)) * 16;
+    const rows_u4 *wp = pack + (size_t)(tn * NBT + nbl) * 6 * 64 + lane;
+    const size_t w_kb = (size_t)nb_all * 6 * 64;
+
+    floatx16 acc[MBW];
+#pragma unroll
+    for (int m = 0; m < MBW; ++m)
+#pragma unroll
+        for (int i = 0; i < 16; ++i) acc[m][i] = 0.f;
+    rows_u4 wc[6];
+#pragma unroll
+    for (int i = 0; i < 6; ++i) wc[i] = rows_u4{0u, 0u, 0u, 0u};
+
+    for (int kb = -1; kb < nkb; ++kb) {
+        const bool more = kb + 1 < nkb;
+        rows_f4 ra[UNITS][ASrc::RAW];
+        rows_u4 wn[6];
+        if (more) {
+            src.fetch(kb + 1, ra);
+#pragma unroll
+            for (int i = 0; i < 6; ++i) wn[i] = wp[(kb + 1) * w_kb + i * 64];
+        }
+        if (kb >= 0) {
+            const unsigned char *buf = smem_rows + (kb & 1) * STAGE + lane * 16;
+#pragma unroll
+            for (int s = 0; s < 2; ++s) {
+                const bf16x8 w1 = __builtin_bit_cast(bf16x8, wc[3 * s]), w2 = __builtin_bit_cast(bf16x8, wc[3 * s + 1]),
+                               w3 = __builtin_bit_cast(bf16x8, wc[3 * s + 2]);
+                bf16x8 a1[MBW], a2[MBW], a3[MBW];
+#pragma unroll
+                for (int m = 0; m < MBW; ++m) {
+                    const unsigned char *af = buf + ((mb0 + m) * 2 + s) * 3 * GR_FRAG;
+                    a1[m] = *reinterpret_cast<const bf16x8 *>(af);
+                    a2[m] = *reinterpret_cast<const bf16x8 *>(af + GR_FRAG);
+                    a3[m] = *reinterpret_cast<const bf16x8 *>(af + 2 * GR_FRAG);
+                }
+                split_mfma6<MBW>(w1, w2, w3, a1, a2, a3, acc);
+            }
+        }
+        if (more) {
+            unsigned char *nxt = smem_rows + ((kb + 1) & 1) * STAGE + a_wr;
+#pragma unroll
+            for (int u = 0; u < UNITS; ++u) {
+                float v[8];
+                src.values(u, kb + 1, ra, v);
+                bf16x8 q1, q2, q3;
+                split8(v, q1, q2, q3);
+                *reinterpret_cast<bf16x8 *>(nxt + u * 12 * GR_FRAG) = q1;
+                *reinterpret_cast<bf16x8 *>(nxt + u * 12 * GR_FRAG + GR_FRAG) = q2;
+                *reinterpret_cast<bf16x8 *>(nxt + u * 12 * GR_FRAG + 2 * GR_FRAG) = q3;
+            }
+#pragma unroll
+            for (int i = 0; i < 6; ++i) wc[i] = wn[i];
+        }
+        __syncthreads();
+    }
+
+    const int n0 = (tn * NBT + nbl) * 32 + 4 * h;
+    rows_f4 b4[4];
+    if (bias) {
+#pragma unroll
+        for (int g = 0; g < 4; ++g) b4[g] = *reinterpret_cast<const rows_f4 *>(bias + n0 + 8 * g);
+    }
+#pragma unroll
+    for (int m = 0; m < MBW; ++m) {
+        float *orow = out + (tm * TM + (mb0 + m) * 32 + r) * (long)N + n0;
+#pragma unroll
+        for (int g = 0; g < 4; ++g) {
+            rows_f4 y;
+#pragma unroll
+            for (int e = 0; e < 4; ++e) y[e] = acc[m][4 * g + e];
+            if (bias) y = y + b4[g];
+            if (relu) {
+#pragma unroll
+                for (int e = 0; e < 4; ++e) y[e] = relu_keep_nan(y[e]);
+            }
+            *reinterpret_cast<rows_f4 *>(orow + 8 * g) = y;
+        }
+    }
+}
+
+}
diff --git a/ws3d_amd/csrc/qinterp_row.h b/ws3d_amd/csrc/qinterp_row.h
--- /dev/null
+++ b/ws3d_amd/csrc/qinterp_row.h
@@ -0,0 +1,37 @@
+#pragma once
+#include "common.h"
+
+namespace ws3d {
+
+__device__ __forceinline__ float4 interp3(float w0, const float4 p0, float w1, const float4 p1, float w2, const float4 p2) {
+    return make_float4(__builtin_fmaf(w2, p2.x, __builtin_fmaf(w0, p0.x, w1 * p1.x)), __builtin_fmaf(w2, p2.y, __builtin_fmaf(w0, p0.y, w1 * p1.y)),
+                       __builtin_fmaf(w2, p2.z, __builtin_fmaf(w0, p0.z, w1 * p1.z)), __builtin_fmaf(w2, p2.w, __builtin_fmaf(w0, p0.w, w1 * p1.w)));
+}
+__device__ __forceinline__ float4 ld4(const float *p) { return *reinterpret_cast<const float4 *>(p); }
+__device__ __forceinline__ void add4(float4 &y, const float4 a) { y.x += a.x; y.y += a.y; y.z += a.z; y.w += a.w; }
+__device__ __forceinline__ void fma4(float4 &y, float s, const float4 a) {
+    y.x = __builtin_fmaf(s, a.x, y.x); y.y = __builtin_fmaf(s, a.y, y.y); y.z = __builtin_fmaf(s, a.z, y.z); y.w = __builtin_fmaf(s, a.w, y.w);
+}
+__device__ __forceinline__ void relu4(float4 &y) { y.x = y.x < 0.f ? 0.f : y.x; y.y = y.y < 0.f ? 0.f : y.y; y.z = y.z < 0.f ? 0.f : y.z; y.w = y.w < 0.f ? 0.f : y.w; }
+
+__device__ __forceinline__ float4 qrow_f4_of(int k, int o, const float4 p0, const float4 p1, const float4 p2, float w0, float w1, float w2, bool has_lin,
+                                             const float4 lv, const float *srow, int c1, const float *__restrict__ wb, const float *__restrict__ bias,
+                                             int relu) {
+    float4 y = interp3(w0, p0, w1, p1, w2, p2);
+    if (has_lin) {
+        add4(y, lv);
+    } else {
+        for (int j = 0; j < c1; ++j) fma4(y, srow[j], ld4(wb + (long)j * o + k));
+        if (bias) add4(y, ld4(bias + k));
+    }
+    if (relu) relu4(y);
+    return y;
+}
+
+__device__ __forceinline__ float4 qrow_f4(int k, int o, const float *q0, const float *q1, const float *q2, float w0, float w1, float w2,
+                                          const float *lrow, const float *srow, int c1, const float *__restrict__ wb, const float *__restrict__ bias, int relu) {
+    return qrow_f4_of(k, o, ld4(q0 + k), ld4(q1 + k), ld4(q2 + k), w0, w1, w2, lrow != nullptr, lrow ? ld4(lrow + k) : make_float4(0.f, 0.f, 0.f, 0.f), srow, c1,
+                      wb, bias, relu);
+}
+
+}
diff --git a/ws3d_amd/fastpath.py b/ws3d_amd/fastpath.py
--- a/ws3d_amd/fastpath.py
+++ b/ws3d_amd/fastpath.py
@@ -68,6 +68,7 @@
 SPLIT_GEMMS = True
 FUSED_GATHER_GEMM2 = True
 BIN_INPUT_AHEAD = True
+SPLIT_QINTERP_GEMM = True
 FUSED_QINTERP_GEMM_MIN_ROWS = 30000
 FUSED_COMPACT3_MAX_LDS = 64 * 1024
 FUSED_GATHER_GEMM = True
@@ -120,6 +121,13 @@
 def _split_gemm(x2d: torch.Tensor, holder, key: str, wt: torch.Tensor, bias=None, relu: bool = False):
     if not SPLIT_GEMMS or x2d.dim() != 2 or not _split_gemm_wins(x2d.size(0), wt.size(0), wt.size(1)):
         return None
+    pack = _gemm_rows_pack_of(holder, key, wt)
+    if pack is None:
+        return None
+    return _C.gemm_rows_split(x2d, pack, wt.size(1), bias, relu)
+
+
+def _gemm_rows_pack_of(holder, key: str, wt: torch.Tensor):
     packs = holder.__dict__.get("_gemm_rows_packs")
     ent = None if packs is None else packs.get(key)
     if ent is None or ent[0] is not wt:
@@ -127,9 +135,13 @@
             return None
         ent = (wt, _C.gemm_rows_pack(wt))
         holder.__dict__.setdefault("_gemm_rows_packs", {})[key] = ent
-    if ent[1] is None:
+    return ent[1]
+
+
+def _fused_pack(block, wt: torch.Tensor, rows: int):
+    if not (SPLIT_GEMMS and SPLIT_QINTERP_GEMM) or not _split_gemm_wins(rows, wt.size(0), wt.size(1)):
         return None
-    return _C.gemm_rows_split(x2d, ent[1], wt.size(1), bias, relu)
+    return _gemm_rows_pack_of(block, "row", wt)
 
 
 def gemm_rows_packs(model):
@@ -609,17 +621,25 @@
         fuse2 = len(blocks) == 2 and B * n >= FUSED_QINTERP_GEMM_MIN_ROWS
         if fuse2:
             wt2, b2, r2 = _row_weights(blocks[1])
+            pack2 = _fused_pack(blocks[1], wt2, B * n)
+
+        def fused(**first):
+            if not fuse2:
+                return None
+            y = _C.qinterp_gemm(q, idx, weight, wt2, b2, r2, relu=r1, pack=pack2, **first) if pack2 is not None else None
+            return y if y is not None else _C.qinterp_gemm(q, idx, weight, wt2, b2, r2, relu=r1, **first)
+
         if c1 > 4:
             lin = _split_gemm(unknown_feats.reshape(B * n, c1), blocks[0], "wb", wb, b1)
             if lin is None:
                 lin = torch.mm(unknown_feats.reshape(B * n, c1), wb) if b1 is None else torch.addmm(b1, unknown_feats.reshape(B * n, c1), wb)
-            y = _C.qinterp_gemm(q, idx, weight, wt2, b2, r2, lin=lin, relu=r1) if fuse2 else None
+            y = fused(lin=lin)
             if y is not None:
                 return y.view(B, n, -1)
             y = _C.qinterp_rows(q, idx, weight, lin=lin, relu=r1)
         else:
             sk = None if c1 == 0 else unknown_feats.contiguous()
-            y = _C.qinterp_gemm(q, idx, weight, wt2, b2, r2, skip=sk, wb=wb if c1 else None, bias=b1, relu=r1) if fuse2 else None
+            y = fused(skip=sk, wb=wb if c1 else None, bias=b1)
             if y is not None:
                 return y.view(B, n, -1)
             y = _C.qinterp_rows(q, idx, weight, skip=sk, wb=wb if c1 else None, bias=b1, relu=r1)
```

After: 7150, median of 6. About the same (+0.9%).
